# saurabh260918/Graph-Attention-Network-GATv2-

Hardware: AMD Instinct MI355X
Metric: edges/sec (fwd+bwd, 2-layer 8-head GATv2) (higher is better)
Workload: dtype f32; 1 GPU; products-shape synthetic power-law graph, 2450000 nodes / 61900000 edges / 100 feat / 47 classes, 2-layer GATv2 heads [8, 8] outdims [8, 8], fp32; launch=eager, parallelism=single GPU, generator=device (csrc/gat_synth.hip), bit-for-bit synth.py

## Files before the change

graph-attention-network-gatv2-_amd/csrc/gat_abi.hip:

```cpp
#include "gat_internal.h"

#include <algorithm>
#include <cmath>
#include <cstdlib>
#include <cstring>
#include <memory>
#include <mutex>

namespace gat {

static thread_local std::string g_err;
void set_error(const std::string& msg) { g_err = msg; }
int fail(int code, const std::string& msg) {
    g_err = msg;
    return code ? code : GAT_E_INVALID;
}
static std::mutex g_choice_mu;
static std::vector<std::pair<std::string, std::string>> g_choices;
const char* choice_env(const char* name) {
    const char* e = getenv(name);
    if (e) {
        std::lock_guard<std::mutex> lock(g_choice_mu);
        bool seen = false;
        for (auto& kv : g_choices) if (kv.first == name) { kv.second = e; seen = true; }
// ... 318 lines not shown
    if (c->drop_step) return 0;
    GAT_TRY(dalloc(c, &c->drop_step, 1));
    GAT_HIP(hipMemsetAsync(c->drop_step, 0, sizeof(uint64_t), c->stream));
    GAT_HIP(hipStreamSynchronize(c->stream));
    return 0;
}
static int32_t ldX_of(gat_ctx* c, int l) { return l == 0 ? c->ld0 : c->layers[l].F; }
static int upload_rows_padded(gat_ctx* c, float* dst, const float* src, int64_t n_rows, int32_t in_dim, hipMemcpyKind kind) {
    if (c->ld0 == in_dim) {
        GAT_HIP(hipMemcpyAsync(dst, src, (size_t)n_rows * in_dim * sizeof(float), kind, c->stream));
        return 0;
    }
    GAT_HIP(hipMemsetAsync(dst, 0, (size_t)n_rows * c->ld0 * sizeof(float), c->stream));
    GAT_HIP(hipMemcpy2DAsync(dst, (size_t)c->ld0 * sizeof(float), src, (size_t)in_dim * sizeof(float), (size_t)in_dim * sizeof(float), (size_t)n_rows, kind, c->stream));
    return 0;
}
static float* gPL_of(gat_ctx* c, int l) { return (c->ov_active && (l & 1)) ? c->gPL_alt : c->gPL; }
static float* gPR_of(gat_ctx* c, int l) { return (c->ov_active && (l & 1)) ? c->gPR_alt : c->gPR; }

static int ensure_drop_buffers(gat_ctx* c) {
    if (!c->buffers_ready || c->drop_pf <= 0.f) return 0;
    const int L = c->cfg.num_layers;
    if (c->xdrop.empty()) {
        c->xdrop.assign((size_t)L, nullptr);
        for (int l = 0; l < L; ++l) GAT_TRY(dalloc(c, &c->xdrop[(size_t)l], c->n_rows * (l == 0 ? c->ld0 : c->layers[l].F)));
    }
    if (c->Xtab && !c->xdrop_tab) GAT_TRY(dalloc(c, &c->xdrop_tab, c->n_table * c->ld0));
    return 0;
}
static int ensure_buffers(gat_ctx* c) {
    if (c->buffers_ready) return 0;
    if (!(c->have_graph && c->have_x && c->have_labels)) return 0;
    const int L = c->cfg.num_layers;
    const int64_t N = c->n_rows, E = c->n_edges, T = c->n_table;
    for (int l = 0; l < L; ++l) {
        Layer& y = c->layers[l];
        if (bf16(c) && !edge_fast_path(y.H, y.D, T))
            return fail(GAT_E_UNSUPPORTED, "bf16 storage needs every layer on the wave-per-row path (H*D in {8,16,32,64}, D a power of two)");
        if (!y.PL_bound) GAT_TRY(dmalloc(c, (void**)&y.PL, (size_t)(T * y.HD * st_bytes(c))));
        GAT_TRY(dalloc(c, &y.PR, N * y.HD));
        if (c->cfg.keep_taps || !edge_fast_path(y.H, y.D, c->n_table)) GAT_TRY(dalloc(c, &y.alpha, E * y.H));
        GAT_TRY(dalloc(c, &y.hpre, N * y.HD));
        GAT_TRY(dalloc(c, &y.hout, N * (l == L - 1 ? y.D : y.HD)));
        if (l < L - 1 || c->cfg.flat_lrelu_index) GAT_TRY(dalloc(c, &y.g, N * y.HD));
        GAT_TRY(dalloc(c, &y.mstat, N * y.H));
        GAT_TRY(dalloc(c, &y.zstat, N * y.H));
        if (c->cfg.keep_taps) {
            GAT_TRY(dalloc(c, &y.ge, E * y.H));
            GAT_TRY(dalloc(c, &y.score, E * y.H));
            GAT_TRY(dalloc(c, &y.galpha, E * y.H));
        }
    }
    if (!c->gPL_bound) GAT_TRY(dalloc(c, &c->gPL, T * c->HDmax));
    GAT_TRY(dalloc(c, &c->gPR, N * c->HDmax));
    if (!c->cfg.flat_lrelu_index) {
        const Layer& yl = c->layers[L - 1];
        const int w = edge_stash_words(yl.H, yl.D);
        c->gh_stride = (w > 0 && w <= 32 && yl.D <= 8 && !bf16(c) && !c->cfg.keep_taps) ? 16 : yl.D;
        GAT_TRY(dalloc(c, &c->gH, N * c->gh_stride));
    }
    GAT_TRY(dalloc(c, &c->items, std::max<int64_t>(c->work.n_items, 1)));
    GAT_TRY(dalloc(c, &c->slot_info, std::max<int32_t>(c->work.n_slots + c->work.n_split, 1)));
    GAT_TRY(dalloc(c, &c->part_acc, (int64_t)std::max<int32_t>(c->work.n_slots, 1) * c->HDmax));
    GAT_TRY(dalloc(c, &c->part_mz, (int64_t)std::max<int32_t>(c->work.n_slots, 1) * 2 * c->Hmax));
    if (c->work.n_items > 0)
        GAT_HIP(hipMemcpyAsync(c->items, c->work.items.data(), c->work.items.size() * sizeof(int32_t),
                               hipMemcpyHostToDevice, c->stream));
    if (c->work.n_slots > 0)
        GAT_HIP(hipMemcpyAsync(c->slot_info, c->work.slot_info.data(), c->work.slot_info.size() * sizeof(int32_t),
                               hipMemcpyHostToDevice, c->stream));
    GAT_HIP(hipStreamSynchronize(c->stream));
    int32_t msg_hd = 0, stash_words = 0;
    const char* no_stash = choice_env("GAT_BWD_STASH");
    for (int l = 0; l < L; ++l) {
        Layer& y = c->layers[l];
        if (!edge_fast_path(y.H, y.D, c->n_table)) continue;
        const int w = edge_stash_words(y.H, y.D);
        y.stash = w > 0 && !c->cfg.keep_taps && !(no_stash && no_stash[0] == '0') && !(bf16(c) && y.HD < 64);
        if (y.stash) stash_words = std::max(stash_words, w); else msg_hd = std::max(msg_hd, y.HD);
    }
    const char* force = choice_env("GAT_BWD_ATOMICS");
    if ((msg_hd > 0 || stash_words > 0) && E > 0 && !(force && force[0] == '1')) {
        float* m = nullptr;
        int32_t *src_ptr = nullptr, *cdst = nullptr, *csrc = nullptr;
        if (hipMalloc((void**)&m, std::max<size_t>((size_t)(E + kPullPad) * msg_hd * (size_t)st_bytes(c), (size_t)(E + kPullPad) * stash_words * sizeof(uint32_t))) == hipSuccess) {
            c->owned.push_back(m);
            if (msg_hd > 0) { c->msg = m; c->msg_hd = msg_hd; }
            if (stash_words > 0) {
                c->stash = reinterpret_cast<uint32_t*>(m); c->stash_words = stash_words;
                if (msg_hd == 0) { c->msg = m; c->msg_hd = 0; }
                GAT_TRY(dalloc(c, &c->gfull, N * c->HDmax));
                if (c->layers[L - 1].stash && c->gH != nullptr && c->gh_stride == 16) c->hbits = reinterpret_cast<uint8_t*>(c->gH) + 32;
                GAT_TRY(dalloc(c, &cdst, E + kPullPad));
                GAT_HIP(hipMemsetAsync(cdst + E, 0, (size_t)kPullPad * sizeof(int32_t), c->stream));
                GAT_HIP(hipMemsetAsync(reinterpret_cast<uint32_t*>(m) + (size_t)E * stash_words, 0, (size_t)kPullPad * stash_words * sizeof(uint32_t), c->stream));
            }
            GAT_TRY(dalloc(c, &c->csc_pos, E));
            GAT_TRY(dalloc(c, &src_ptr, T + 1));
            static const int run_env = [] { const char* e = choice_env("GAT_PULL_RUN"); return e ? atoi(e) : -1; }();
            const int32_t run = run_env >= 0 ? (run_env / 32) * 32 : 64;
            if (run > 0) GAT_TRY(dalloc(c, &csrc, E + kPullPad));
            GAT_TRY(build_csc(c->col_idx, E, T, c->csc_pos, src_ptr, csrc, c->stream));
            if (cdst) GAT_TRY(build_csc_dst(c->row_ptr, c->csc_pos, cdst, N, E, c->stream));
            SourceIndex& ix = c->src_index;
            ix.src_ptr = src_ptr; ix.cdst = cdst; ix.n_table = T; ix.n_slots = E; ix.slot_capacity = E + kPullPad;
            HeavyList hl;
            GAT_TRY(build_heavy_list(src_ptr, T, E, &hl, c->stream, run));
            auto upload = [&](auto** d, const std::vector<int32_t>& h, int per) -> int {
                GAT_TRY(dalloc(c, d, std::max<int64_t>((int64_t)(h.size() / per), 1)));
                if (!h.empty()) GAT_HIP(hipMemcpyAsync(*d, h.data(), h.size() * sizeof(int32_t), hipMemcpyHostToDevice, c->stream));
                return 0;
            };
            if (hl.run > 0 && csrc != nullptr) {
                ix.run = hl.run; ix.n_runs = hl.n_runs; ix.n_open = (int32_t)(hl.open.size() / 4); ix.n_empty = (int64_t)hl.empty.size();
                int4* d_open = nullptr; int32_t* d_empty = nullptr;
                GAT_TRY(upload(&d_open, hl.open, 4));
                GAT_TRY(upload(&d_empty, hl.empty, 1));
                GAT_TRY(dalloc(c, &ix.run_part, std::max<int64_t>(2 * ix.n_runs, 1) * c->HDmax));
                GAT_HIP(hipStreamSynchronize(c->stream));
                ix.open = d_open; ix.empty = d_empty; ix.csrc = csrc;
            }
            ix.n_chunks = (int32_t)(hl.chunks.size() / 4); ix.n_heavy = (int32_t)(hl.heavy.size() / 4);
            if (c->stash != nullptr && !hl.items.empty()) {
                int4* d_items = nullptr;
                GAT_TRY(upload(&d_items, hl.items, 4));
                GAT_HIP(hipStreamSynchronize(c->stream));
                ix.items = d_items; ix.n_items = (int64_t)(hl.items.size() / 4);
            }
            if (ix.n_heavy > 0) {
                int4* d_chunks = nullptr; int4* d_heavy = nullptr;
                GAT_TRY(upload(&d_chunks, hl.chunks, 4));
                GAT_TRY(upload(&d_heavy, hl.heavy, 4));
                GAT_TRY(dalloc(c, &ix.part, (int64_t)ix.n_chunks * c->HDmax));
                GAT_HIP(hipStreamSynchronize(c->stream));
                ix.chunks = d_chunks; ix.heavy = d_heavy;
            }
        } else {
            (void)hipGetLastError();
            for (int l = 0; l < L; ++l) c->layers[l].stash = false;
        }
    } else {
        for (int l = 0; l < L; ++l) c->layers[l].stash = false;
    }
    GAT_TRY(dalloc(c, &c->ga_partial, (int64_t)L * kGaPartialRows * c->HDmax));
    int64_t gw = 0;
    c->gw_off.assign((size_t)L, 0);
    for (int l = 0; l < L; ++l) { c->gw_off[(size_t)l] = gw; gw += grad_w_scratch_floats(N, c->layers[l].F, c->layers[l].HD); }
    gw = std::max<int64_t>(gw, 1);
    if (c->Xtab) gw = std::max(gw, grad_w_scratch_floats(T, c->layers[0].F, c->layers[0].HD));
    for (int l = 0; l < L; ++l) {
        const Layer& y = c->layers[l];
        if (l == 0 && c->Xtab) gw = std::max({gw, project_scratch_floats(T, y.F, y.HD, kPartLeft), project_scratch_floats(N, y.F, y.HD, kPartRight)});
        else gw = std::max(gw, project_scratch_floats(N, y.F, y.HD, kPartBoth));
    }
    GAT_TRY(dalloc(c, &c->gw_scratch, gw));
    c->gw_scratch_floats = gw;
    const int C = c->cfg.num_classes, DL = c->layers[L - 1].D;
    const int64_t NH = head_rows(c);
    GAT_TRY(dalloc(c, &c->hb_partial, (int64_t)head_bwd_blocks(NH, C, DL) * C * DL));
    GAT_TRY(dalloc(c, &c->loss_partial, head_blocks(NH)));
    GAT_TRY(dalloc(c, &c->correct_partial, head_blocks(NH)));
    GAT_TRY(dalloc(c, &c->loss_out, 1));
    GAT_TRY(dalloc(c, &c->correct_out, 1));
    GAT_TRY(dalloc(c, &c->y, NH * C));
    if (res_route(c)) {
        if (norm_on(c)) GAT_TRY(dalloc(c, &c->norm_partial, (int64_t)L * 2 * kResPartialRows * c->HDmax));
        GAT_TRY(dalloc(c, &c->resG, N * c->HDmax));
        GAT_TRY(dalloc(c, &c->res_agg, N * c->HDmax));
        GAT_TRY(dalloc(c, &c->res_partial, (int64_t)L * kResPartialRows * c->HDmax));
        if (c->group_cnt[GAT_PARAM_WRES]) {
            int64_t rg = 0;
            c->res_gw_off.assign((size_t)L, 0);
            for (int l = 0; l < L; ++l) {
                GAT_TRY(dalloc(c, &c->layers[l].R, N * c->layers[l].HD));
                c->res_gw_off[(size_t)l] = rg;
                rg += grad_w_scratch_floats(N, c->layers[l].F, c->layers[l].HD);
            }
            GAT_TRY(dalloc(c, &c->res_gw_scratch, std::max<int64_t>(rg, 1)));
        }
        GAT_TRY(ensure_drop_step(c));
    }
    if (edge_feat_on(c)) {
        const int64_t Ea = std::max<int64_t>(E, 1);
        int64_t wg = 0;
        c->we_gw_off.assign((size_t)L, 0);
        for (int l = 0; l < L; ++l) {
            GAT_TRY(dalloc(c, &c->layers[l].PE, Ea * c->layers[l].HD));
            c->we_gw_off[(size_t)l] = wg;
// ... 574 lines not shown
    }
    float* own_rows = reinterpret_cast<float*>(reinterpret_cast<char*>(y.PL) + c->table_row0 * y.HD * st_bytes(c));
    return launch_project(Xin_of(c, l), W_of(c, l), own_rows, y.PR, c->n_rows, y.F, y.HD, kPartBoth, bf16(c), c->gw_scratch, c->gw_scratch_floats, c->stream, ldX_of(c, l));
}

static EdgeFwdArgs plan_forward_edges(gat_ctx* c, int32_t l);
int gat_layer_forward_edges(gat_ctx* c, int32_t l) {
    GAT_TRY(check_layer(c, l));
    GAT_TRY(check_edge_features(c));
    const EdgeFwdArgs a = plan_forward_edges(c, l);
    EdgeFwdExtras x;
    x.drop = drop_args(c, l); x.res = c->layers[l].R; x.bias = b_of(c, l); x.ln = ln_args(c, l); x.pe = c->layers[l].PE;
    Scope t(c, GAT_K_EDGE_FWD);
    return launch_edge_forward(a, c->stream, &x);
}
static EdgeFwdArgs plan_forward_edges(gat_ctx* c, int32_t l) {
    Layer& y = c->layers[l];
    EdgeFwdArgs a{};
    a.row_ptr = c->row_ptr; a.col_idx = c->col_idx; a.PL = y.PL; a.PR = y.PR; a.a = a_of(c, l);
    a.alpha = y.alpha; a.score = y.score; a.hpre = y.hpre; a.hout = y.hout; a.mstat = y.mstat; a.zstat = y.zstat;
    a.n_rows = c->n_rows; a.n_table = c->n_table; a.bf16 = bf16(c); a.H = y.H; a.D = y.D; a.is_last = (l == c->cfg.num_layers - 1);
    a.slope = c->cfg.negative_slope;
    a.items = c->items; a.n_items = c->work.n_items; a.slot_info = c->slot_info; a.n_slots = c->work.n_slots; a.n_split = c->work.n_split;
    a.part_acc = c->part_acc; a.part_mz = c->part_mz;
    return a;
}

static int readout_pool(gat_ctx* c) {
    if (!readout_on(c)) return 0;
    const Layer& y = c->layers.back();
    ReadoutFwdArgs a{};
    a.x = y.hout; a.x_stride = y.D; a.graph_ptr = c->ro_graph_ptr;
    a.items = c->ro_items; a.n_items = c->ro_n_items; a.split = c->ro_split; a.n_split = c->ro_n_split;
    a.pooled = c->ro_P; a.argmax = c->ro_argmax; a.part = c->ro_part; a.part_arg = c->ro_part_arg;
    a.width = y.D; a.mode = c->readout_mode;
    Scope t(c, GAT_K_HEAD_FWD);
    return launch_readout_forward(a, c->stream);
}
static int readout_unpool(gat_ctx* c) {
    if (!readout_on(c)) return 0;
    ReadoutBwdArgs a{};
    a.gpooled = c->ro_gP; a.argmax = c->ro_argmax; a.graph_ptr = c->ro_graph_ptr; a.node_graph = c->ro_node_graph;
    a.gh = c->gH; a.gh_stride = c->gh_stride; a.n_rows = c->n_rows;
    a.width = c->layers.back().D; a.mode = c->readout_mode;
    Scope t(c, GAT_K_HEAD_BWD);
    return launch_readout_backward(a, c->stream);
}
static void head_args(gat_ctx* c, HeadArgs* f, HeadBwdArgs* b);
static LossHeadArgs loss_head_args(gat_ctx* c);
int gat_head_forward(gat_ctx* c, float* loss_sum, int32_t* n_correct) {
    GAT_TRY(check_layer(c, 0));
    HeadArgs a{}; HeadBwdArgs unused{};
    head_args(c, &a, &unused);
    GAT_TRY(readout_pool(c));
    {
        Scope t(c, GAT_K_HEAD_FWD);
        if (c->loss_mode != 0) GAT_TRY(launch_loss_head_forward(loss_head_args(c), c->stream));
        else GAT_TRY(launch_head_forward(a, c->stream));
    }
    c->y_valid = true;
    if (loss_sum || n_correct) {
        float hl = 0.f; int32_t hc = 0;
        GAT_HIP(hipMemcpyAsync(&hl, c->loss_out, sizeof(float), hipMemcpyDeviceToHost, c->stream));
        GAT_HIP(hipMemcpyAsync(&hc, c->correct_out, sizeof(int32_t), hipMemcpyDeviceToHost, c->stream));
        GAT_HIP(hipStreamSynchronize(c->stream));
        if (loss_sum) *loss_sum = hl;
        if (n_correct) *n_correct = hc;
    }
    return 0;
}

int gat_head_backward(gat_ctx* c) {
    GAT_TRY(check_layer(c, 0));
    HeadArgs unused{}; HeadBwdArgs a{};
    head_args(c, &unused, &a);
    {
        Scope t(c, GAT_K_HEAD_BWD);
        if (c->loss_mode != 0) GAT_TRY(launch_loss_head_grad(loss_head_args(c), false, c->stream));
        else GAT_TRY(launch_head_backward(a, c->stream));
    }
    return readout_unpool(c);
}

struct BwdPlan { EdgeBwdArgs a; bool store, stash, last_g; DropArgs drop; };
static int plan_backward_edges(gat_ctx* c, int32_t l, BwdPlan* P) {
    Layer& y = c->layers[l];
    const bool store = c->msg != nullptr && edge_fast_path(y.H, y.D, c->n_table);
    const bool stash = store && y.stash && c->stash != nullptr;
    EdgeBwdArgs a{};
    a.row_ptr = c->row_ptr; a.col_idx = c->col_idx; a.PL = y.PL; a.PR = y.PR; a.a = a_of(c, l);
    a.alpha = y.alpha; a.mstat = y.mstat; a.zstat = y.zstat;
    a.hpre = y.hpre; a.g = y.g; a.gPL = gPL_of(c, l); a.gPR = gPR_of(c, l); a.ge = y.ge; a.galpha = y.galpha;
    a.g_raw = l < c->cfg.num_layers - 1;
    a.gh = (l == c->cfg.num_layers - 1) ? c->gH : nullptr; a.gh_stride = c->gh_stride; a.hb_stride = 64;
    if (res_route(c)) {
        a.g = c->resG; a.g_raw = 0; a.gh = nullptr; a.hpre = c->res_agg;
    }
    a.pos = store ? c->csc_pos : nullptr; a.msg = store ? c->msg : nullptr;
    a.stash = stash ? c->stash : nullptr; a.gfull = stash ? c->gfull : nullptr; a.stash_spare = (uint32_t)c->n_edges;
    static const int pull_last = [] { const char* e = choice_env("GAT_PULL_LAST"); return e ? (e[0] == '0' ? 0 : 1) : -1; }();
    const bool runs_form = c->src_index.csrc != nullptr && short_lists_take_runs(c->n_edges, c->n_table);
    const bool big_rows = (int64_t)c->n_rows * y.H * y.D * 4 > ((int64_t)(runs_form ? 64 : 128) << 20);
    const bool last_g = stash && a.gh != nullptr && c->hbits != nullptr && !bf16(c) && !edge_feat_on(c) && (pull_last >= 0 ? pull_last == 1 : big_rows) &&
                        c->n_rows < ((int64_t)1 << 26);
    a.hbits = last_g ? c->hbits : nullptr;
    a.items = c->items; a.n_items = c->work.n_items; a.slot_info = c->slot_info; a.n_slots = c->work.n_slots; a.n_split = c->work.n_split;
    a.part_acc = c->part_acc;
    a.dbg = c->dbg;
    a.ga_partial = c->ga_partial + (int64_t)l * kGaPartialRows * c->HDmax; a.n_rows = c->n_rows; a.n_table = c->n_table; a.bf16 = bf16(c); a.H = y.H; a.D = y.D;
    a.slope = c->cfg.negative_slope;
    P->drop = drop_args(c, l);
    a.ga_blocks = edge_backward_blocks(a, &P->drop, y.PE != nullptr);
    P->a = a; P->store = store; P->stash = stash; P->last_g = last_g;
    return 0;
}
static int sum_backward_edges(gat_ctx* c, int32_t l, const BwdPlan& P) {
    Layer& y = c->layers[l];
    if (!P.stash && !P.store) return 0;
    Scope t(c, GAT_K_GPL_SUM);
    if (P.stash) {
        const PullArgs p{c->stash, c->gfull, bf16(c), P.last_g ? c->gH : nullptr, P.last_g ? c->hbits : nullptr, c->gh_stride, 64,
                         a_of(c, l), c->cfg.negative_slope, gPL_of(c, l), y.H, y.D};
        return launch_gpl_pull(c->src_index, p, c->stream);
    }
    return launch_gpl_sum(c->src_index, c->msg, bf16(c), gPL_of(c, l), y.HD, c->stream);
}
static int res_backward_layer(gat_ctx* c, int32_t l) {
    Layer& y = c->layers[l];
    const bool last = l == c->cfg.num_layers - 1;
    ResBwdArgs r{};
    r.hpre = y.hpre; r.g = y.g; r.gh = (last && c->gH != nullptr) ? c->gH : nullptr; r.res = y.R; r.bias = b_of(c, l);
    r.G = c->resG; r.agg = c->res_agg;
    r.partial = b_of(c, l) ? c->res_partial + (int64_t)l * kResPartialRows * c->HDmax : nullptr;
    r.n_rows = c->n_rows; r.H = y.H; r.D = y.D; r.gh_stride = c->gh_stride; r.g_raw = last ? 0 : 1;
    r.slope = c->cfg.negative_slope;
    Scope t(c, GAT_K_MISC);
    if (norm_layer(c, l)) {
        NormBwdArgs n{};
        n.gamma = lng_of(c, l); n.beta = lnb_of(c, l); n.eps = c->norm_eps;
        n.part_gamma = c->norm_partial + (int64_t)l * 2 * kResPartialRows * c->HDmax;
        n.part_beta = n.part_gamma + (int64_t)kResPartialRows * c->HDmax;
        r.blocks = norm_backward_blocks(c->n_rows, y.HD);
        n.r = r;
        GAT_TRY(launch_norm_backward(n, c->stream));
        GAT_TRY(launch_reduce_partials_add(n.part_gamma, r.blocks, y.HD, glng_of(c, l), c->stream));
        GAT_TRY(launch_reduce_partials_add(n.part_beta, r.blocks, y.HD, glnb_of(c, l), c->stream));
    } else {
        r.blocks = res_backward_blocks(c->n_rows, y.HD);
        GAT_TRY(launch_res_backward(r, c->stream));
    }
    if (r.partial != nullptr) return launch_reduce_partials_add(r.partial, r.blocks, y.HD, gb_of(c, l), c->stream);
    return 0;
}
int gat_layer_backward_edges(gat_ctx* c, int32_t l) {
    GAT_TRY(check_layer(c, l));
    GAT_TRY(check_edge_features(c));
    Layer& y = c->layers[l];
    BwdPlan P;
    GAT_TRY(plan_backward_edges(c, l, &P));
    if (res_route(c)) GAT_TRY(res_backward_layer(c, l));
    if (!P.store) {
        Scope t(c, GAT_K_MISC);
        GAT_HIP(hipMemsetAsync(gPL_of(c, l), 0, (size_t)c->n_table * y.HD * sizeof(float), c->stream));
    }
    {
        Scope t(c, GAT_K_EDGE_BWD);
        GAT_TRY(launch_edge_backward(P.a, c->stream, &P.drop, y.PE, y.PE != nullptr ? c->gPE : nullptr));
    }
    GAT_TRY(sum_backward_edges(c, l, P));
    Scope t(c, GAT_K_MISC);
    return launch_reduce_partials_add(P.a.ga_partial, P.a.ga_blocks, y.HD, ga_of(c, l), c->stream);
}

static int backward_grad_w(gat_ctx* c, int32_t l, hipStream_t st) {
    Layer& y = c->layers[l];
    const float* gPL_rows = gPL_of(c, l) + c->table_row0 * y.HD;
    Scope t(c, GAT_K_GRAD_W, st);
    if (y.R != nullptr)
        GAT_TRY(launch_grad_wres(c->resG, Xin_of(c, l), gWres_of(c, l), c->res_gw_scratch + c->res_gw_off[(size_t)l], c->n_rows, y.F, y.HD, st, ldX_of(c, l)));
    if (y.PE != nullptr)
        GAT_TRY(launch_grad_wres(c->gPE, c->EA, gWe_of(c, l), c->we_gw_scratch + c->we_gw_off[(size_t)l], c->n_edges, c->edge_dim, y.HD, st, c->ea_ld));
    if (l == 0 && c->Xtab) {
        GAT_TRY(launch_grad_w(gPL_of(c, l), nullptr, Xtab_of(c), gW_of(c, l), c->gw_scratch, c->n_table, y.F, y.HD, kPartLeft, st, c->ld0));
        return launch_grad_w(nullptr, gPR_of(c, l), Xin_of(c, 0), gW_of(c, l), c->gw_scratch, c->n_rows, y.F, y.HD, kPartRight, st, c->ld0);
    }
    return launch_grad_w(gPL_rows, gPR_of(c, l), Xin_of(c, l), gW_of(c, l), c->gw_scratch + c->gw_off[(size_t)l], c->n_rows, y.F, y.HD, kPartBoth, st, ldX_of(c, l));
}
static int backward_grad_x(gat_ctx* c, int32_t l) {
    if (l == 0) return 0;
    Layer& y = c->layers[l];
    const float* gPL_rows = gPL_of(c, l) + c->table_row0 * y.HD;
    Scope t(c, GAT_K_GRAD_X);
    GAT_TRY(launch_grad_x(gPL_rows, gPR_of(c, l), W_of(c, l), nullptr, c->layers[l - 1].g, c->n_rows, y.F, y.HD,
                          c->cfg.negative_slope, c->stream));
    if (y.R != nullptr) GAT_TRY(launch_grad_x_res(c->resG, Wres_of(c, l), c->layers[l - 1].g, c->n_rows, y.F, y.HD, c->stream));
    if (feat_drop_on(c)) return launch_feat_drop_bwd(c->layers[l - 1].g, c->n_rows, y.F, drop_args(c, l, kDropFeat), c->stream);
    return 0;
}
int gat_layer_backward_dense(gat_ctx* c, int32_t l) {
    GAT_TRY(check_layer(c, l));
    GAT_TRY(check_edge_features(c));
    GAT_TRY(backward_grad_w(c, l, c->stream));
    return backward_grad_x(c, l);
}

// ... 1164 lines not shown
```

graph-attention-network-gatv2-_amd/csrc/gat_csc.hip:

```cpp
#include "gat_internal.h"

#include <hipcub/hipcub.hpp>
#include <utility>

namespace gat {
namespace {

__global__ __launch_bounds__(256) void iota_kernel(int32_t* v, int64_t n) {
    const int64_t stride = (int64_t)gridDim.x * blockDim.x;
    for (int64_t i = (int64_t)blockIdx.x * blockDim.x + threadIdx.x; i < n; i += stride) v[i] = (int32_t)i;
}
__global__ __launch_bounds__(256) void invert_perm_kernel(const int32_t* __restrict__ perm, int32_t* __restrict__ pos,
                                                         int64_t n) {
    const int64_t stride = (int64_t)gridDim.x * blockDim.x;
    for (int64_t i = (int64_t)blockIdx.x * blockDim.x + threadIdx.x; i < n; i += stride) pos[perm[i]] = (int32_t)i;
}
__global__ __launch_bounds__(256) void segment_offsets_kernel(const int32_t* __restrict__ keys, int64_t n_keys,
                                                             int32_t* __restrict__ ptr, int64_t n_seg) {
    const int64_t stride = (int64_t)gridDim.x * blockDim.x;
    for (int64_t s = (int64_t)blockIdx.x * blockDim.x + threadIdx.x; s <= n_seg; s += stride) {
        int64_t lo = 0, hi = n_keys;
        while (lo < hi) {
            const int64_t mid = (lo + hi) >> 1;
            if ((int64_t)keys[mid] < s) lo = mid + 1; else hi = mid;
// ... 226 lines not shown
}

template <int HD>
__global__ __launch_bounds__(256) void gpl_sum_bf16_group_kernel(const int32_t* __restrict__ src_ptr,
                                                                 const float* __restrict__ msg, float* __restrict__ gPL,
                                                                 int64_t n_table, int32_t kHeavySlots) {
    constexpr int LPR = HD / 8, RPI = 64 / LPR, U = 4;
    const int lane = threadIdx.x & 63;
    const int wave = __builtin_amdgcn_readfirstlane(threadIdx.x >> 6);
    const int q = lane % LPR, r = lane / LPR;
    const int64_t s = ((int64_t)blockIdx.x * 4 + wave) * RPI + r;
    int b = 0, e = 0;
    if (s < n_table) { b = src_ptr[s]; e = src_ptr[s + 1]; }
    const bool heavy = (e - b) > kHeavySlots;
    const bool big = !heavy && (e - b) > kGroupMax;
    const uint4* m8 = reinterpret_cast<const uint4*>(msg);
    float acc[8];
#pragma unroll
    for (int k = 0; k < 8; ++k) acc[k] = 0.f;
    auto add = [&](float (&a8)[8], const uint4& v) {
        const uint32_t w[4] = {v.x, v.y, v.z, v.w};
#pragma unroll
        for (int k = 0; k < 4; ++k) {
            a8[2 * k] += __builtin_bit_cast(float, w[k] << 16);
            a8[2 * k + 1] += __builtin_bit_cast(float, w[k] & 0xFFFF0000u);
        }
    };
    if (!big && !heavy) {
        for (int i0 = b; i0 < e; i0 += U) {
            uint4 v[U];
#pragma unroll
            for (int u = 0; u < U; ++u)
                v[u] = (i0 + u < e) ? m8[(int64_t)(i0 + u) * LPR + q] : make_uint4(0u, 0u, 0u, 0u);
#pragma unroll
            for (int u = 0; u < U; ++u) add(acc, v[u]);
        }
    }
    uint64_t todo = __ballot(big && q == 0);
    while (todo) {
        const int g = (__ffsll((unsigned long long)todo) - 1) / LPR;
        todo &= todo - 1;
        const int bg = __shfl(b, g * LPR), eg = __shfl(e, g * LPR);
        float t[8];
#pragma unroll
        for (int k = 0; k < 8; ++k) t[k] = 0.f;
        for (int i0 = bg; i0 < eg; i0 += RPI * U) {
            uint4 v[U];
#pragma unroll
            for (int u = 0; u < U; ++u) {
                const int i = i0 + u * RPI + r;
                v[u] = (i < eg) ? m8[(int64_t)i * LPR + q] : make_uint4(0u, 0u, 0u, 0u);
            }
#pragma unroll
            for (int u = 0; u < U; ++u) add(t, v[u]);
        }
#pragma unroll
        for (int off = LPR; off < 64; off <<= 1)
#pragma unroll
            for (int k = 0; k < 8; ++k) t[k] += __shfl_xor(t[k], off);
        if (r == g) {
#pragma unroll
            for (int k = 0; k < 8; ++k) acc[k] = t[k];
        }
    }
    if (s < n_table && !heavy) {
        float4* out = reinterpret_cast<float4*>(gPL + s * HD + q * 8);
        out[0] = make_float4(acc[0], acc[1], acc[2], acc[3]);
        out[1] = make_float4(acc[4], acc[5], acc[6], acc[7]);
    }
}

template <int N> struct PullVec;
template <> struct PullVec<2> { typedef float T __attribute__((ext_vector_type(2))); };
template <> struct PullVec<4> { typedef float T __attribute__((ext_vector_type(4))); };

template <class T>
__device__ __forceinline__ void stream_store(T* p, const T& v) {
#ifdef GAT_NT_STORES
    __builtin_nontemporal_store(v, p);
#else
    *p = v;
#endif
}
template <int HD, int N, bool BF, int LASTD>
__device__ __forceinline__ typename PullVec<N>::T pull_range(const uint32_t* __restrict__ stash,
                                                             const int32_t* __restrict__ cdst,
                                                             const float* __restrict__ gfull, const uint8_t* __restrict__ hbits, int gh_stride, int hb_stride,
                                                             float slope, int b, int e, int lane,
                                                             typename PullVec<N>::T ac, typename PullVec<N>::T acs) {
    using V = typename PullVec<N>::T;
    constexpr int LPE = HD / N, G = 64 / LPE;
    constexpr int CH = 16, U = CH / G;
    static_assert(U >= 1, "lane layout");
    const int cp = lane % LPE, gidx = lane / LPE;
    V acc;
#pragma unroll
    for (int i = 0; i < N; ++i) acc[i] = 0.f;
    auto load_dst = [&](int i0) {
        const int j = i0 + (lane & (CH - 1));
        return cdst[j < e ? j : e - 1];
    };
    int dv = load_dst(b);
    for (int i0 = b; i0 < e; i0 += CH) {
        const int dn = (i0 + CH < e) ? load_dst(i0 + CH) : 0;
        uint32_t w[U];
        V g[U];
#pragma unroll
        for (int u = 0; u < U; ++u) {
            const int i = i0 + u * G + gidx;
            const int ic = i < e ? i : e - 1;
            w[u] = stash[(uint64_t)(uint32_t)ic * LPE + cp];
            const uint32_t drow = (uint32_t)__shfl(dv, u * G + gidx);
            if constexpr (LASTD > 0) {
                constexpr float inv_heads = 1.0f / (float)(HD / LASTD);
                const V gh4 = *reinterpret_cast<const V*>(gfull + (size_t)drow * gh_stride + (cp * N) % LASTD);
                const uint32_t nib = hbits[(size_t)drow * hb_stride + cp];
#pragma unroll
                for (int k = 0; k < N; ++k) g[u][k] = gh4[k] * ((nib >> k) & 1u ? 1.0f : slope) * inv_heads;
            } else if constexpr (BF) {
                const char* p = reinterpret_cast<const char*>(gfull) + drow * (uint32_t)(HD * 2) + (uint32_t)cp * (uint32_t)(N * 2);
                if constexpr (N == 2) {
                    const uint32_t w2 = *reinterpret_cast<const uint32_t*>(p);
                    g[u][0] = __builtin_bit_cast(float, w2 << 16); g[u][1] = __builtin_bit_cast(float, w2 & 0xFFFF0000u);
                } else {
                    const uint2 w2 = *reinterpret_cast<const uint2*>(p);
                    g[u][0] = __builtin_bit_cast(float, w2.x << 16); g[u][1] = __builtin_bit_cast(float, w2.x & 0xFFFF0000u);
                    g[u][2] = __builtin_bit_cast(float, w2.y << 16); g[u][3] = __builtin_bit_cast(float, w2.y & 0xFFFF0000u);
                }
            } else {
                const uint32_t off = drow * (uint32_t)(HD * 4) + (uint32_t)cp * (uint32_t)(N * 4);
#ifdef GAT_NT_GATHER
                g[u] = __builtin_nontemporal_load(reinterpret_cast<const V*>(reinterpret_cast<const char*>(gfull) + off));
#else
                g[u] = *reinterpret_cast<const V*>(reinterpret_cast<const char*>(gfull) + off);
#endif
            }
        }
#pragma unroll
        for (int u = 0; u < U; ++u) {
            const int i = i0 + u * G + gidx;
            const float val = __builtin_bit_cast(float, w[u] & ~((1u << N) - 1u));
            const float oth = __shfl_xor(val, 1);
            const float al = (cp & 1) ? oth : val, ge = (cp & 1) ? val : oth;
            V asel;
#pragma unroll
            for (int k = 0; k < N; ++k) asel[k] = (w[u] >> k) & 1u ? ac[k] : acs[k];
            const float keep = i < e ? 1.0f : 0.0f;
            acc += (g[u] * al + asel * ge) * keep;
        }
        dv = dn;
    }
#pragma unroll
    for (int off = LPE; off < 64; off <<= 1)
#pragma unroll
        for (int k = 0; k < N; ++k) acc[k] += __shfl_xor(acc[k], off);
    return acc;
}

template <int N> struct PullTabs { alignas(16) float m[2][1 << N][N]; };
template <int N>
__device__ __forceinline__ void pull_tabs_init(PullTabs<N>& T, float slope, float inv_heads) {
    for (int t = threadIdx.x; t < 2 * (1 << N) * N; t += blockDim.x) {
        const int tab = t / ((1 << N) * N), nib = (t / N) % (1 << N), k = t % N;
        const float v = (nib >> k) & 1 ? 1.0f : slope;
        T.m[tab][nib][k] = tab ? v * inv_heads : v;
    }
    __syncthreads();
}
template <int K>
__device__ __forceinline__ float select_bit(uint32_t bits, float a, float b) {
    uint32_t mask, sel;
    asm("v_bfe_i32 %0, %1, %2, 1" : "=v"(mask) : "v"(bits), "n"(K));
    asm("v_bfi_b32 %0, %1, %2, %3" : "=v"(sel) : "v"(mask), "v"(__builtin_bit_cast(uint32_t, a)), "v"(__builtin_bit_cast(uint32_t, b)));
    return __builtin_bit_cast(float, sel);
}
template <int N>
__device__ __forceinline__ typename PullVec<N>::T select_bits(uint32_t bits, typename PullVec<N>::T a, typename PullVec<N>::T b) {
    typename PullVec<N>::T r;
    r[0] = select_bit<0>(bits, a[0], b[0]);
    r[1] = select_bit<1>(bits, a[1], b[1]);
    if constexpr (N > 2) { r[2] = select_bit<2>(bits, a[2], b[2]); r[3] = select_bit<3>(bits, a[3], b[3]); }
    return r;
}
template <int HD, int N, int LASTD, bool TAB>
__device__ __forceinline__ typename PullVec<N>::T pull_range2(const PullTabs<N>& T, const uint32_t* __restrict__ stash,
                                                              const int32_t* __restrict__ cdst, const float* __restrict__ gfull,
                                                              const uint8_t* __restrict__ hbits, int b, int e, int lane,
                                                              typename PullVec<N>::T ac, float slope) {
    using V = typename PullVec<N>::T;
    [[maybe_unused]] const V acs = ac * slope;
    [[maybe_unused]] V mhi, mlo;
    if constexpr (LASTD > 0) {
#pragma unroll
        for (int k = 0; k < N; ++k) { mhi[k] = 1.0f / (float)(HD / LASTD); mlo[k] = slope * (1.0f / (float)(HD / LASTD)); }
    }
    constexpr int LPE = HD / N, G = 64 / LPE;
    constexpr int CH = 16, U = CH / G;
    constexpr uint32_t kMask = (1u << N) - 1u;
    static_assert(U >= 1, "lane layout");
    const int cp = lane % LPE, gidx = lane / LPE;
    V acc;
#pragma unroll
    for (int i = 0; i < N; ++i) acc[i] = 0.f;
    const char* sp = reinterpret_cast<const char*>(stash + (uint64_t)(uint32_t)b * LPE);
    const char* dp = reinterpret_cast<const char*>(cdst + b);
    const uint32_t doff = (uint32_t)(lane & (CH - 1)) * 4u;
    int dv = *reinterpret_cast<const int32_t*>(dp + doff);
    for (int rem = e - b; rem > 0; rem -= CH, sp += CH * LPE * 4, dp += CH * 4) {
        const int dn = *reinterpret_cast<const int32_t*>(dp + CH * 4 + doff);
        const int d0 = __builtin_amdgcn_readfirstlane(dv);
        uint32_t w[U];
        V g[U];
#pragma unroll
        for (int u = 0; u < U; ++u) {
            const bool valid = u * G + gidx < rem;
            const uint32_t ww = *reinterpret_cast<const uint32_t*>(sp + (uint32_t)((u * G + gidx) * LPE + cp) * 4u);
            int drow = __shfl(dv, u * G + gidx);
            drow = valid ? drow : d0;
            w[u] = valid ? ww : 0u;
            if constexpr (LASTD > 0) {
                const uint32_t ro = (uint32_t)drow << 6;
                const V gh4 = *reinterpret_cast<const V*>(reinterpret_cast<const char*>(gfull) + (ro + (uint32_t)((cp * N) % LASTD) * 4u));
                const uint32_t nib = *reinterpret_cast<const uint8_t*>(reinterpret_cast<const char*>(hbits) + (ro + (uint32_t)cp));
                if constexpr (TAB) g[u] = gh4 * *reinterpret_cast<const V*>(&T.m[1][nib & kMask][0]);
                else g[u] = gh4 * select_bits<N>(nib, mhi, mlo);
            } else {
                g[u] = *reinterpret_cast<const V*>(reinterpret_cast<const char*>(gfull) + ((uint32_t)drow * (uint32_t)(HD * 4) + (uint32_t)cp * (uint32_t)(N * 4)));
            }
        }
#pragma unroll
        for (int u = 0; u < U; ++u) {
            const float val = __builtin_bit_cast(float, w[u] & ~kMask);
            const float oth = __builtin_bit_cast(float, __builtin_amdgcn_update_dpp(0, __builtin_bit_cast(int, val), 0xB1, 0xF, 0xF, true));
            const float al = (cp & 1) ? oth : val, ge = (cp & 1) ? val : oth;
            acc += g[u] * al;
            if constexpr (TAB) acc += (ac * ge) * *reinterpret_cast<const V*>(&T.m[0][w[u] & kMask][0]);
            else acc += select_bits<N>(w[u], ac, acs) * ge;
        }
        dv = dn;
    }
#pragma unroll
    for (int off = LPE; off < 64; off <<= 1)
#pragma unroll
        for (int k = 0; k < N; ++k) acc[k] += __shfl_xor(acc[k], off);
    return acc;
}

template <int HD, int N, bool BF, int LASTD, int V2 = 0>
__global__ __launch_bounds__(256) void gpl_pull_kernel(const int32_t* __restrict__ src_ptr, const uint32_t* __restrict__ stash,
                                                       const int32_t* __restrict__ cdst, const float* __restrict__ gfull,
                                                       const uint8_t* __restrict__ hbits, int gh_stride, int hb_stride,
                                                       const float* __restrict__ a, float slope, float* __restrict__ gPL,
                                                       int64_t n_table, int32_t kHeavySlots) {
    using V = typename PullVec<N>::T;
    constexpr int LPE = HD / N;
    __shared__ PullTabs<N> tabs;
    if constexpr (V2 == 1) pull_tabs_init<N>(tabs, slope, LASTD > 0 ? 1.0f / (float)(HD / (LASTD > 0 ? LASTD : 1)) : 1.0f);
    const int lane = threadIdx.x & 63;
    const int wave = __builtin_amdgcn_readfirstlane(threadIdx.x >> 6);
    const int64_t s = (int64_t)blockIdx.x * (blockDim.x >> 6) + wave;
    if (s >= n_table) return;
    const int b = __builtin_amdgcn_readfirstlane(src_ptr[s]), e = __builtin_amdgcn_readfirstlane(src_ptr[s + 1]);
    if (e - b > kHeavySlots) return;
    const int cp = lane % LPE;
    V acc;
    if (b < e) {
        const V ac = *reinterpret_cast<const V*>(a + cp * N);
        if constexpr (V2 != 0) acc = pull_range2<HD, N, LASTD, V2 == 1>(tabs, stash, cdst, gfull, hbits, b, e, lane, ac, slope);
        else acc = pull_range<HD, N, BF, LASTD>(stash, cdst, gfull, hbits, gh_stride, hb_stride, slope, b, e, lane, ac, ac * slope);
    } else {
#pragma unroll
        for (int i = 0; i < N; ++i) acc[i] = 0.f;
    }
    if (lane < LPE) stream_store(reinterpret_cast<V*>(gPL + s * HD + cp * N), acc);
}

template <int HD, int N, bool BF, int LASTD, int V2 = 0>
__global__ __launch_bounds__(256) void gpl_pull_chunk_kernel(const int4* __restrict__ chunks, int32_t n_chunks,
                                                             const uint32_t* __restrict__ stash, const int32_t* __restrict__ cdst,
                                                             const float* __restrict__ gfull, const uint8_t* __restrict__ hbits,
                                                             int gh_stride, int hb_stride, const float* __restrict__ a,
                                                             float slope, float* __restrict__ part) {
    using V = typename PullVec<N>::T;
    constexpr int LPE = HD / N;
    __shared__ PullTabs<N> tabs;
    if constexpr (V2 == 1) pull_tabs_init<N>(tabs, slope, LASTD > 0 ? 1.0f / (float)(HD / (LASTD > 0 ? LASTD : 1)) : 1.0f);
    const int lane = threadIdx.x & 63;
    const int wave = __builtin_amdgcn_readfirstlane(threadIdx.x >> 6);
    const int k = blockIdx.x * 4 + wave;
    if (k >= n_chunks) return;
    const int4 ch = chunks[k];
    const int cp = lane % LPE;
    const V ac = *reinterpret_cast<const V*>(a + cp * N);
    V acc;
    if constexpr (V2 != 0) acc = pull_range2<HD, N, LASTD, V2 == 1>(tabs, stash, cdst, gfull, hbits, __builtin_amdgcn_readfirstlane(ch.x), __builtin_amdgcn_readfirstlane(ch.y), lane, ac, slope);
    else acc = pull_range<HD, N, BF, LASTD>(stash, cdst, gfull, hbits, gh_stride, hb_stride, slope, ch.x, ch.y, lane, ac, ac * slope);
    if (lane < LPE) *reinterpret_cast<V*>(part + (int64_t)ch.z * HD + cp * N) = acc;
}

template <int HD, int N, bool BF, int LASTD>
__global__ __launch_bounds__(256) void gpl_pull3_kernel(const int4* __restrict__ items, int64_t n_items,
                                                        const uint32_t* __restrict__ stash, const int32_t* __restrict__ cdst,
                                                        const float* __restrict__ gfull, const uint8_t* __restrict__ hbits,
                                                        int gh_stride, int hb_stride,
                                                        const float* __restrict__ a, float slope, float* __restrict__ gPL,
                                                        float* __restrict__ part) {
    using V = typename PullVec<N>::T;
    constexpr int LPE = HD / N, G = 64 / LPE, U = 4;
    static_assert(LPE >= U, "lane layout");
    const int lane = threadIdx.x & 63;
    const int wave = __builtin_amdgcn_readfirstlane(threadIdx.x >> 6);
    const int cp = lane % LPE, gidx = lane / LPE;
    const int64_t it = ((int64_t)blockIdx.x * (blockDim.x >> 6) + wave) * G + gidx;
    int src = -1, b = 0, e = 0, pslot = -1;
    if (it < n_items) { const int4 item = items[it]; src = item.x; b = item.y; e = item.z; pslot = item.w; }
    const V ac = *reinterpret_cast<const V*>(a + cp * N);
    const V acs = ac * slope;
    V acc;
#pragma unroll
    for (int i = 0; i < N; ++i) acc[i] = 0.f;
    int nst = (e - b + U - 1) / U;
#pragma unroll
    for (int off = LPE; off < 64; off <<= 1) { const int o = __shfl_xor(nst, off); nst = nst > o ? nst : o; }
    nst = __builtin_amdgcn_readfirstlane(nst);
    auto load_dst = [&](int st) {
        int j = b + st * U + (cp & (U - 1));
        j = j < e ? j : e - 1;
        return cdst[j > 0 ? j : 0];
    };
    int dv = load_dst(0);
    for (int st = 0; st < nst; ++st) {
        const int dn = load_dst(st + 1);
        uint32_t w[U];
        V g[U];
#pragma unroll
        for (int u = 0; u < U; ++u) {
            int j = b + st * U + u;
            j = j < e ? j : e - 1;
            j = j > 0 ? j : 0;
            w[u] = stash[(uint64_t)(uint32_t)j * LPE + cp];
            const uint32_t drow = (uint32_t)__shfl(dv, gidx * LPE + u);
            if constexpr (LASTD > 0) {
                constexpr float inv_heads = 1.0f / (float)(HD / LASTD);
                const V gh4 = *reinterpret_cast<const V*>(gfull + (size_t)drow * gh_stride + (cp * N) % LASTD);
                const uint32_t nib = hbits[(size_t)drow * hb_stride + cp];
#pragma unroll
                for (int k = 0; k < N; ++k) g[u][k] = gh4[k] * ((nib >> k) & 1u ? 1.0f : slope) * inv_heads;
            } else if constexpr (BF) {
                const char* p = reinterpret_cast<const char*>(gfull) + drow * (uint32_t)(HD * 2) + (uint32_t)cp * (uint32_t)(N * 2);
                if constexpr (N == 2) {
                    const uint32_t w2 = *reinterpret_cast<const uint32_t*>(p);
                    g[u][0] = __builtin_bit_cast(float, w2 << 16); g[u][1] = __builtin_bit_cast(float, w2 & 0xFFFF0000u);
                } else {
                    const uint2 w2 = *reinterpret_cast<const uint2*>(p);
                    g[u][0] = __builtin_bit_cast(float, w2.x << 16); g[u][1] = __builtin_bit_cast(float, w2.x & 0xFFFF0000u);
                    g[u][2] = __builtin_bit_cast(float, w2.y << 16); g[u][3] = __builtin_bit_cast(float, w2.y & 0xFFFF0000u);
                }
            } else {
                const uint32_t off = drow * (uint32_t)(HD * 4) + (uint32_t)cp * (uint32_t)(N * 4);
#ifdef GAT_NT_GATHER
                g[u] = __builtin_nontemporal_load(reinterpret_cast<const V*>(reinterpret_cast<const char*>(gfull) + off));
#else
                g[u] = *reinterpret_cast<const V*>(reinterpret_cast<const char*>(gfull) + off);
#endif
            }
        }
#pragma unroll
        for (int u = 0; u < U; ++u) {
            const float val = __builtin_bit_cast(float, w[u] & ~((1u << N) - 1u));
            const float oth = __shfl_xor(val, 1);
            const float al = (cp & 1) ? oth : val, ge = (cp & 1) ? val : oth;
            V asel;
#pragma unroll
            for (int k = 0; k < N; ++k) asel[k] = (w[u] >> k) & 1u ? ac[k] : acs[k];
            const float keep = (b + st * U + u < e) ? 1.0f : 0.0f;
            acc += (g[u] * al + asel * ge) * keep;
        }
        dv = dn;
    }
    if (src < 0) return;
    float* dst = pslot < 0 ? gPL + (int64_t)src * HD : part + (int64_t)pslot * HD;
// ... 154 lines not shown
        }
        return;
    }
    const int64_t wv = (int64_t)((int)blockIdx.x - rd.zero_blocks) * 4 + wave;
    const int64_t r = wv * G + gidx;
    const int64_t j0 = r * rd.run, left = rd.n_slots - j0;
    const int cnt = left <= 0 ? 0 : (left < rd.run ? (int)left : rd.run);
    const int nT = (__builtin_amdgcn_readfirstlane(cnt) + SS - 1) / SS;
    if (nT == 0) return;
    const int64_t jb = cnt > 0 ? j0 : 0;
    const int sb = (cnt > 0 && j0 > 0) ? rd.csrc[j0 - 1] : -1;
    const char* mp = reinterpret_cast<const char*>(msg) + ((uint64_t)jb * LPR + q) * 16u;
    int code[K], coden[K], dummy;
#pragma unroll
    for (int k = 0; k < K; ++k) runs_index(rd, nullptr, jb, r, cnt, sb, 0, k * LPR + q, dummy, code[k]);
    for (int T = 0; T < nT; ++T, mp += SS * LPR * 16) {
#pragma unroll
        for (int k = 0; k < K; ++k) coden[k] = 0;
        if (T + 1 < nT) {
#pragma unroll
            for (int k = 0; k < K; ++k) runs_index(rd, nullptr, jb, r, cnt, sb, 0, (T + 1) * SS + k * LPR + q, dummy, coden[k]);
        }
        if (T * SS < cnt) {
            const int rem = cnt - T * SS;
            static_for(std::make_integer_sequence<int, SS / U>{}, [&](auto bc) {
                constexpr int b = decltype(bc)::value;
                uint4 v[U];
                static_for(std::make_integer_sequence<int, U>{}, [&](auto uc) {
                    constexpr int u = decltype(uc)::value, slot = b * U + u;
                    const uint4 vv = *reinterpret_cast<const uint4*>(mp + slot * LPR * 16);
                    v[u] = slot < rem ? vv : make_uint4(0u, 0u, 0u, 0u);
                });
                static_for(std::make_integer_sequence<int, U>{}, [&](auto uc) {
                    constexpr int u = decltype(uc)::value, slot = b * U + u;
                    const uint32_t w[4] = {v[u].x, v[u].y, v[u].z, v[u].w};
                    if constexpr (BF) {
#pragma unroll
                        for (int k = 0; k < 4; ++k) {
                            acc[2 * k] += __builtin_bit_cast(float, w[k] << 16);
                            acc[2 * k + 1] += __builtin_bit_cast(float, w[k] & 0xFFFF0000u);
                        }
                    } else {
#pragma unroll
                        for (int k = 0; k < 4; ++k) acc[k] += __builtin_bit_cast(float, w[k]);
                    }
                    const int cw = group_bcast<slot % LPR, LPR>(code[slot / LPR], gidx);
                    if (cw < 0) {
                        const uint32_t row = (uint32_t)cw & 0x7fffffffu;
                        store_row(row >= (uint32_t)rd.n_table ? rd.part + (size_t)(row - (uint32_t)rd.n_table) * HD : gPL + (size_t)row * HD);
#pragma unroll
                        for (int i = 0; i < CPL; ++i) acc[i] = 0.f;
                    }
                });
            });
        }
#pragma unroll
        for (int k = 0; k < K; ++k) code[k] = coden[k];
    }
}

__global__ __launch_bounds__(256) void gpl_runs_fix_kernel(const int4* __restrict__ open, int32_t n_open, const float* __restrict__ part,
                                                           float* __restrict__ gPL, int32_t Q ) {
    const int64_t t = (int64_t)blockIdx.x * blockDim.x + threadIdx.x;
    const int64_t k = t / Q;
    const int q = (int)(t % Q);
    if (k >= n_open) return;
    const int4 o = open[k];
    const float4* p4 = reinterpret_cast<const float4*>(part);
    float4 acc = p4[(int64_t)(2 * o.y + 1) * Q + q];
    int r = o.y + 1;
    for (; r + 4 <= o.z; r += 4) {
        float4 v[4];
#pragma unroll
        for (int i = 0; i < 4; ++i) v[i] = p4[(int64_t)(2 * (r + i) + 1) * Q + q];
#pragma unroll
        for (int i = 0; i < 4; ++i) { acc.x += v[i].x; acc.y += v[i].y; acc.z += v[i].z; acc.w += v[i].w; }
    }
    for (; r < o.z; ++r) { const float4 v = p4[(int64_t)(2 * r + 1) * Q + q]; acc.x += v.x; acc.y += v.y; acc.z += v.z; acc.w += v.w; }
    { const float4 v = p4[(int64_t)(2 * o.z) * Q + q]; acc.x += v.x; acc.y += v.y; acc.z += v.z; acc.w += v.w; }
    reinterpret_cast<float4*>(gPL)[(int64_t)o.x * Q + q] = acc;
}

__global__ __launch_bounds__(256) void csc_dst_kernel(const int32_t* __restrict__ row_ptr, const int32_t* __restrict__ pos,
                                                     int32_t* __restrict__ cdst, int64_t n_rows, int64_t n_edges) {
    const int64_t stride = (int64_t)gridDim.x * blockDim.x;
    for (int64_t e = (int64_t)blockIdx.x * blockDim.x + threadIdx.x; e < n_edges; e += stride) {
        int64_t lo = 0, hi = n_rows;
        while (hi - lo > 1) {
            const int64_t mid = (lo + hi) >> 1;
            if ((int64_t)row_ptr[mid] <= e) lo = mid; else hi = mid;
        }
        cdst[pos[e]] = (int32_t)lo;
    }
}

}

int build_csc_dst(const int32_t* row_ptr, const int32_t* pos, int32_t* cdst, int64_t n_rows, int64_t n_edges, hipStream_t s) {
    if (n_edges <= 0) return 0;
    const int64_t blocks = std::min<int64_t>((n_edges + 255) / 256, 65536);
    hipLaunchKernelGGL(csc_dst_kernel, dim3((unsigned)blocks), dim3(256), 0, s, row_ptr, pos, cdst, n_rows, n_edges);
    GAT_HIP(hipGetLastError());
    return 0;
}

static int pull_runs_env() {
    static const int v = [] { const char* e = choice_env("GAT_PULL_RUNS"); return e ? (e[0] == '0' ? 0 : 1) : -1; }();
    return v;
}
static int pull_groups_env() {
    static const int v = [] { const char* e = choice_env("GAT_PULL_GROUPS"); return e ? (e[0] == '1' ? 1 : 0) : -1; }();
    return v;
}
static int pull_u_env() {
    static const int v = [] { const char* e = choice_env("GAT_PULL_U"); return e ? atoi(e) : 0; }();
    return v;
}
static int pull_v2_env() {
    static const int v = [] { const char* e = choice_env("GAT_PULL_V2"); return e ? atoi(e) : -1; }();
    return v;
}
static int gpl_waves_env() {
    static const int v = [] { const char* e = choice_env("GAT_GPL_WAVES"); const int w = e ? atoi(e) : 0; return (w == 1 || w == 2 || w == 4) ? w : 0; }();
    return v;
}
static int gpl_group_env() {
    static const int v = [] { const char* e = choice_env("GAT_GPL_GROUP"); return e ? (e[0] == '1' ? 1 : 0) : -1; }();
    return v;
}
static int gpl_bf16_group_env() {
    static const int v = [] { const char* e = choice_env("GAT_GPL_BF16_GROUP"); return e ? (e[0] == '0' ? 0 : 1) : -1; }();
    return v;
}

namespace {
struct GplPick {
    enum Form { kLists, kItems, kRuns };
    const void* fn = nullptr;
    Form form = kLists;
    const void* chunk_fn = nullptr;
    unsigned grid = 0, block = 256;
    RunsDev rd{};
};
#define GAT_K(...) ((const void*)(__VA_ARGS__))

static GplPick pick_runs(const SourceIndex& ix, const void* fn, int G) {
    GplPick p{fn, GplPick::kRuns};
    RunsDev& rd = p.rd;
    rd.csrc = ix.csrc; rd.empty = ix.empty; rd.part = ix.run_part; rd.n_empty = ix.n_empty; rd.n_slots = ix.n_slots; rd.n_table = ix.n_table;
    rd.run = ix.run; rd.zero_blocks = (int32_t)((ix.n_empty + 4 * G * 8 - 1) / (4 * G * 8));
    const int64_t waves = (ix.n_runs + G - 1) / G;
    p.grid = (unsigned)(rd.zero_blocks + (waves + 3) / 4);
    return p;
}

template <int HD, int N, bool BF, int LASTD>
GplPick pick_pull(const SourceIndex& ix, const PullArgs& A, bool padded) {
    constexpr int LPE = HD / N, G = 64 / LPE;
    const int wpb = gpl_waves_env() ? gpl_waves_env() : 1;
    const int runs_env = pull_runs_env(), groups_env = pull_groups_env();
    const bool records64 = LASTD == 0 || (A.gh_stride == 16 && A.hb_stride == 64);
    const bool runs_ok = padded && ix.csrc != nullptr && ix.run % LPE == 0 && records64;
    if (runs_ok && (runs_env >= 0 ? runs_env == 1 : (groups_env < 0 && short_lists_take_runs(ix.n_slots, ix.n_table)))) {
        constexpr int U = LPE % 8 == 0 ? 8 : 4;
        const int u_env = pull_u_env();
        if constexpr (LPE == 16 && !BF) {
            if (u_env == 4) return pick_runs(ix, GAT_K(gpl_pull_runs_kernel<HD, N, BF, LASTD, 4>), G);
            if (u_env == 16) return pick_runs(ix, GAT_K(gpl_pull_runs_kernel<HD, N, BF, LASTD, 16>), G);
        }
        return pick_runs(ix, GAT_K(gpl_pull_runs_kernel<HD, N, BF, LASTD, U>), G);
    }
    const bool groups = groups_env >= 0 ? groups_env == 1 : (ix.n_slots < 8 * ix.n_table && ix.n_items >= 32768);
    if (ix.items != nullptr && groups) {
        const int64_t quads = (ix.n_items + G - 1) / G;
        return {GAT_K(gpl_pull3_kernel<HD, N, BF, LASTD>), GplPick::kItems, nullptr, (unsigned)((quads + 3) / 4)};
    }
    const int v2_env = pull_v2_env();
    const int v2_want = v2_env >= 0 ? v2_env : (LASTD > 0 ? 2 : 0);
    const int v2 = (padded && !BF && records64) ? v2_want : 0;
    const unsigned grid = (unsigned)((ix.n_table + wpb - 1) / wpb), block = 64u * wpb;
    if constexpr (!BF) {
        if (v2 == 1) return {GAT_K(gpl_pull_kernel<HD, N, BF, LASTD, 1>), GplPick::kLists, GAT_K(gpl_pull_chunk_kernel<HD, N, BF, LASTD, 1>), grid, block};
        if (v2 == 2) return {GAT_K(gpl_pull_kernel<HD, N, BF, LASTD, 2>), GplPick::kLists, GAT_K(gpl_pull_chunk_kernel<HD, N, BF, LASTD, 2>), grid, block};
    }
    return {GAT_K(gpl_pull_kernel<HD, N, BF, LASTD, 0>), GplPick::kLists, GAT_K(gpl_pull_chunk_kernel<HD, N, BF, LASTD, 0>), grid, block};
}

template <int HD>
GplPick pick_sum(const SourceIndex& ix, bool bf) {
    const int runs_env = pull_runs_env();
    const bool group_env = gpl_group_env() >= 0 || gpl_bf16_group_env() >= 0;
    if (ix.csrc != nullptr && ix.run % 16 == 0 &&
        (runs_env >= 0 ? runs_env == 1 : (!group_env && !bf && short_lists_take_runs(ix.n_slots, ix.n_table))))
        return pick_runs(ix, bf ? GAT_K(gpl_sum_runs_kernel<HD, true>) : GAT_K(gpl_sum_runs_kernel<HD, false>), 64 / (HD / (bf ? 8 : 4)));
    const int wpb = gpl_waves_env() ? gpl_waves_env() : 4;
    const unsigned wgrid = (unsigned)((ix.n_table + wpb - 1) / wpb), wblock = 64u * wpb;
    const int rpi = 64 / (HD / (bf ? 8 : 4));
    const unsigned ggrid = (unsigned)((ix.n_table + 4 * rpi - 1) / (4 * rpi));
    if (bf) {
        const void* chunk = GAT_K(gpl_chunk_kernel<HD, true>);
        if (gpl_bf16_group_env() != 0) return {GAT_K(gpl_sum_bf16_group_kernel<HD>), GplPick::kLists, chunk, ggrid};
        return {GAT_K(gpl_sum_bf16_kernel<HD>), GplPick::kLists, chunk, wgrid, wblock};
    }
    const void* chunk = GAT_K(gpl_chunk_kernel<HD, false>);
    const int force = gpl_group_env();
    const bool group = force >= 0 ? force == 1 : ix.n_slots < 8 * ix.n_table;
    if (group) return {GAT_K(gpl_sum_group_kernel<HD>), GplPick::kLists, chunk, ggrid};
    return {GAT_K(gpl_sum_kernel<HD>), GplPick::kLists, chunk, wgrid, wblock};
}

}

static GplPick pick_pull_pass(const SourceIndex& ix, const PullArgs& A, bool last, bool padded) {
#define GAT_PULL_SHAPE(HD_, N_, D_)                                                                      \
    case HD_ * 1000 + D_:                                                                                \
        if (last) return pick_pull<HD_, N_, false, D_>(ix, A, padded);                                   \
        return A.g_bf16 ? pick_pull<HD_, N_, true, 0>(ix, A, padded) : pick_pull<HD_, N_, false, 0>(ix, A, padded);
    switch (A.H * A.D * 1000 + A.D) {
        GAT_PULL_SHAPE(64, 4, 8) GAT_PULL_SHAPE(32, 4, 8) GAT_PULL_SHAPE(64, 2, 4) GAT_PULL_SHAPE(32, 2, 4) GAT_PULL_SHAPE(16, 2, 4) GAT_PULL_SHAPE(8, 2, 4)
        default: return {};
    }
#undef GAT_PULL_SHAPE
}
static GplPick pick_sum_pass(const SourceIndex& ix, int32_t HD, bool bf) {
    switch (HD) {
        case 64: return pick_sum<64>(ix, bf);
        case 32: return pick_sum<32>(ix, bf);
        case 16: return pick_sum<16>(ix, bf);
        case 8: return pick_sum<8>(ix, bf);
        default: return {};
    }
}

static int run_pick(const SourceIndex& ix, const GplPick& p, void** args, void** chunk_args, float* gPL, int32_t HD, hipStream_t s) {
    const bool heavy = p.form != GplPick::kRuns && ix.n_heavy > 0;
    auto heavy_fix = [&] {
        const int64_t threads = (int64_t)ix.n_heavy * HD;
        hipLaunchKernelGGL(gpl_heavy_fix_kernel, dim3((unsigned)((threads + 255) / 256)), dim3(256), 0, s, ix.heavy, ix.n_heavy, ix.part, gPL, HD);
    };
    if (heavy && p.chunk_fn != nullptr) {
        GAT_HIP(hipLaunchKernel(p.chunk_fn, dim3((unsigned)((ix.n_chunks + 3) / 4)), dim3(256), chunk_args, 0, s));
        heavy_fix();
    }
    if (p.grid > 0) GAT_HIP(hipLaunchKernel(p.fn, dim3(p.grid), dim3(p.block), args, 0, s));
    if (heavy && p.chunk_fn == nullptr) heavy_fix();
    if (p.form == GplPick::kRuns && ix.n_open > 0) {
        const int64_t threads = (int64_t)ix.n_open * (HD / 4);
        hipLaunchKernelGGL(gpl_runs_fix_kernel, dim3((unsigned)((threads + 255) / 256)), dim3(256), 0, s, ix.open, ix.n_open, ix.run_part, gPL, HD / 4);
    }
    GAT_HIP(hipGetLastError());
    return 0;
}

int launch_gpl_pull(const SourceIndex& ix, const PullArgs& A, hipStream_t s) {
    if (ix.n_table <= 0) return 0;
    const bool padded = ix.slot_capacity >= ix.n_slots + kPullPad;
    const bool last = A.gh != nullptr && A.hbits != nullptr;
    GplPick p = pick_pull_pass(ix, A, last, padded);
    if (p.fn == nullptr) return fail(GAT_E_UNSUPPORTED, "gpl_pull: no stash path for this (H, D)");
    SourceIndex x = ix;
    PullArgs q = A;
    const float* g = last ? A.gh : A.gfull;
    int32_t hs = heavy_slots(ix.n_slots);
    void* lists[] = {&x.src_ptr, &q.stash, &x.cdst, &g, &q.hbits, &q.gh_stride, &q.hb_stride, &q.a, &q.slope, &q.gPL, &x.n_table, &hs};
    void* chunk[] = {&x.chunks, &x.n_chunks, &q.stash, &x.cdst, &g, &q.hbits, &q.gh_stride, &q.hb_stride, &q.a, &q.slope, &x.part};
    void* items[] = {&x.items, &x.n_items, &q.stash, &x.cdst, &g, &q.hbits, &q.gh_stride, &q.hb_stride, &q.a, &q.slope, &q.gPL, &x.part};
    void* runs[] = {&q.stash, &x.cdst, &g, &q.hbits, &q.a, &q.slope, &q.gPL, &p.rd};
    return run_pick(ix, p, p.form == GplPick::kRuns ? runs : p.form == GplPick::kItems ? items : lists, chunk, A.gPL, A.H * A.D, s);
}

int build_csc(const int32_t* col_idx, int64_t n_edges, int64_t n_table, int32_t* pos, int32_t* src_ptr,
              int32_t* csrc, hipStream_t s) {
    if (csrc) GAT_HIP(hipMemsetAsync(csrc + std::max<int64_t>(n_edges, 0), 0xFF, (size_t)kPullPad * sizeof(int32_t), s));
    if (n_edges <= 0) {
        GAT_HIP(hipMemsetAsync(src_ptr, 0, (size_t)(n_table + 1) * sizeof(int32_t), s));
        return 0;
    }
    int32_t *iota = nullptr, *keys_out = nullptr, *perm = nullptr;
    void* temp = nullptr;
    size_t temp_bytes = 0;
    int end_bit = 1;
    while (((int64_t)1 << end_bit) < n_table) ++end_bit;
    int rc = 0;
    auto cleanup = [&]() { (void)hipFree(iota); (void)hipFree(keys_out); (void)hipFree(perm); (void)hipFree(temp); };
#define CSC_HIP(x) do { hipError_t e__ = (x); if (e__ != hipSuccess) { cleanup(); return fail((int)e__, std::string(#x) + ": " + hipGetErrorString(e__)); } } while (0)
    CSC_HIP(hipMalloc((void**)&iota, n_edges * sizeof(int32_t)));
    CSC_HIP(hipMalloc((void**)&keys_out, n_edges * sizeof(int32_t)));
    CSC_HIP(hipMalloc((void**)&perm, n_edges * sizeof(int32_t)));
    int64_t blocks = std::min<int64_t>((n_edges + 255) / 256, 65536);
    hipLaunchKernelGGL(iota_kernel, dim3((unsigned)blocks), dim3(256), 0, s, iota, n_edges);
    CSC_HIP(hipcub::DeviceRadixSort::SortPairs(nullptr, temp_bytes, col_idx, keys_out, iota, perm, (int)n_edges, 0,
                                               end_bit, s));
    CSC_HIP(hipMalloc(&temp, temp_bytes));
    CSC_HIP(hipcub::DeviceRadixSort::SortPairs(temp, temp_bytes, col_idx, keys_out, iota, perm, (int)n_edges, 0,
                                               end_bit, s));
    hipLaunchKernelGGL(invert_perm_kernel, dim3((unsigned)blocks), dim3(256), 0, s, perm, pos, n_edges);
    if (csrc) CSC_HIP(hipMemcpyAsync(csrc, keys_out, (size_t)n_edges * sizeof(int32_t), hipMemcpyDeviceToDevice, s));
    const int64_t sblocks = std::min<int64_t>((n_table + 1 + 255) / 256, 65536);
    hipLaunchKernelGGL(segment_offsets_kernel, dim3((unsigned)sblocks), dim3(256), 0, s, keys_out, n_edges, src_ptr,
                       n_table);
    CSC_HIP(hipGetLastError());
    CSC_HIP(hipStreamSynchronize(s));
#undef CSC_HIP
    cleanup();
    return rc;
}

int build_heavy_list(const int32_t* d_src_ptr, int64_t n_table, int64_t n_edges, HeavyList* out, hipStream_t s, int32_t run) {
    out->chunks.clear(); out->heavy.clear();
    out->run = 0; out->n_runs = 0; out->open.clear(); out->empty.clear();
    if (n_table <= 0) return 0;
    std::vector<int32_t> ptr((size_t)n_table + 1);
    GAT_HIP(hipMemcpyAsync(ptr.data(), d_src_ptr, ptr.size() * sizeof(int32_t), hipMemcpyDeviceToHost, s));
    GAT_HIP(hipStreamSynchronize(s));
    if (run > 0 && n_table + 2 * ((n_edges + run - 1) / run) + 2 < 0x7fffffffLL) {
        out->run = run; out->n_runs = (n_edges + run - 1) / run;
        for (int64_t src = 0; src < n_table; ++src) {
            const int32_t b = ptr[(size_t)src], e = ptr[(size_t)src + 1];
            if (e == b) { out->empty.push_back((int32_t)src); continue; }
            const int32_t r0 = b / run, r1 = (e - 1) / run;
            if (r0 != r1) out->open.insert(out->open.end(), {(int32_t)src, r0, r1, 0});
        }
    }
    const int kHeavySlots = heavy_slots(n_edges);
    out->threshold = kHeavySlots;
    out->items.clear();
    for (int64_t src = 0; src < n_table; ++src) {
        const int32_t b = ptr[(size_t)src], e = ptr[(size_t)src + 1];
        if (e - b <= kHeavySlots) continue;
        const int32_t first = (int32_t)(out->chunks.size() / 4);
        int32_t n = 0;
        for (int32_t cb = b; cb < e; cb += kHeavySlots, ++n) {
            out->chunks.insert(out->chunks.end(), {cb, std::min(e, cb + kHeavySlots), first + n, 0});
            out->items.insert(out->items.end(), {(int32_t)src, cb, std::min(e, cb + kHeavySlots), first + n});
        }
        out->heavy.insert(out->heavy.end(), {(int32_t)src, first, n, 0});
    }
    {
        const int64_t win = 4096;
        std::vector<int64_t> cnt((size_t)kHeavySlots + 2);
        for (int64_t s0 = 0; s0 < n_table; s0 += win) {
            const int64_t s1 = std::min(n_table, s0 + win);
            std::fill(cnt.begin(), cnt.end(), 0);
            for (int64_t sr = s0; sr < s1; ++sr) { const int32_t d = ptr[(size_t)sr + 1] - ptr[(size_t)sr]; if (d <= kHeavySlots) ++cnt[(size_t)(kHeavySlots - d) + 1]; }
            for (size_t i = 1; i < cnt.size(); ++i) cnt[i] += cnt[i - 1];
            const size_t base = out->items.size();
            out->items.resize(base + 4 * (size_t)cnt.back());
            for (int64_t sr = s0; sr < s1; ++sr) {
// ... 24 lines not shown
```

graph-attention-network-gatv2-_amd/csrc/gat_edge_kernels.hip:

```cpp
#include "gat_internal.h"

#include <algorithm>
#include <map>
#include <mutex>
#include <utility>

namespace gat {
namespace {

constexpr float kLog2e = 1.4426950408889634f;
constexpr float kLn2 = 0.6931471805599453f;

__device__ __forceinline__ float lrelu(float v, float s) { return v > 0.f ? v : v * s; }
__device__ __forceinline__ float exp2_fast(float x) { return __builtin_amdgcn_exp2f(x); }
__device__ __forceinline__ float attn_keep(const DropArgs& d, uint32_t kd, int k, int h) {
    return drop_factor(d, drop_mix(drop_mix(kd, (uint32_t)k), (uint32_t)h));
}
__device__ __forceinline__ uint32_t edge_row_key(const DropArgs& d, int64_t row) { return drop_mix(drop_edge_key(d), drop_node(d, row)); }
struct RowKeys { uint32_t kd, ke; int rb; };
__device__ __forceinline__ void row_keys(const DropArgs& d, int64_t row, const int32_t* row_ptr, RowKeys& k) {
    k.kd = drop_mix(drop_key(d, kDropAttn), drop_node(d, row)); k.rb = row_ptr[row]; k.ke = edge_row_key(d, row);
}
__device__ __forceinline__ float pe_load(const float* __restrict__ pe, int j, int HD, int c) { return pe[(int64_t)j * HD + c]; }
template <bool EXT> struct FwdArgsOf { typedef EdgeFwdArgs T; };
// ... 458 lines not shown
        }
#pragma unroll
        for (int off = HD; off < 64; off <<= 1) gpr += __shfl_xor(gpr, off);
        if (gidx == 0) {
            if (slot < 0) A.gPR[row * HD + c] = gpr;
            else A.part_acc[(int64_t)slot * HD + c] = gpr;
        }
    }
#pragma unroll
    for (int off = HD; off < 64; off <<= 1) ga += __shfl_xor(ga, off);
    if (gidx == 0) red[wave][c] = ga;
    __syncthreads();
    if (threadIdx.x < HD)
        A.ga_partial[(int64_t)blockIdx.x * HD + threadIdx.x] =
            (red[0][threadIdx.x] + red[1][threadIdx.x]) + (red[2][threadIdx.x] + red[3][threadIdx.x]);
}

template <int N> struct VecOf;
template <> struct VecOf<2> { typedef float T __attribute__((ext_vector_type(2))); };
template <> struct VecOf<4> { typedef float T __attribute__((ext_vector_type(4))); };
template <int N> using vnf = typename VecOf<N>::T;

template <int N> __device__ __forceinline__ vnf<N> vzero() {
    vnf<N> r;
#pragma unroll
    for (int i = 0; i < N; ++i) r[i] = 0.f;
    return r;
}
template <int N> __device__ __forceinline__ float hsum(vnf<N> v) {
    if constexpr (N == 2) return v[0] + v[1];
    else return (v[0] + v[1]) + (v[2] + v[3]);
}
template <int N> __device__ __forceinline__ vnf<N> lrelu_n(vnf<N> s, float slope) {
    const vnf<N> t = s * slope;
    vnf<N> r;
#pragma unroll
    for (int i = 0; i < N; ++i) r[i] = fmaxf(s[i], t[i]);
    return r;
}
template <int N> __device__ __forceinline__ vnf<N> select_pos(vnf<N> s, vnf<N> a, vnf<N> b) {
    vnf<N> r;
#pragma unroll
    for (int i = 0; i < N; ++i) r[i] = s[i] > 0.f ? a[i] : b[i];
    return r;
}
template <int N> __device__ __forceinline__ vnf<N> shfl_xor_n(vnf<N> v, int off) {
    vnf<N> r;
#pragma unroll
    for (int i = 0; i < N; ++i) r[i] = __shfl_xor(v[i], off);
    return r;
}

template <int HD, int N, bool BF>
__device__ __forceinline__ vnf<N> gather_row_n(const float* __restrict__ table, int row, int cp) {
    if constexpr (BF) {
        const uint32_t off = (uint32_t)row * (uint32_t)(HD * 2) + (uint32_t)cp * (uint32_t)(N * 2);
        const char* p = reinterpret_cast<const char*>(table) + off;
        vnf<N> r;
        if constexpr (N == 2) {
            const uint32_t w = *reinterpret_cast<const uint32_t*>(p);
            r[0] = __builtin_bit_cast(float, w << 16); r[1] = __builtin_bit_cast(float, w & 0xFFFF0000u);
        } else {
            const uint2 w = *reinterpret_cast<const uint2*>(p);
            r[0] = __builtin_bit_cast(float, w.x << 16); r[1] = __builtin_bit_cast(float, w.x & 0xFFFF0000u);
            r[2] = __builtin_bit_cast(float, w.y << 16); r[3] = __builtin_bit_cast(float, w.y & 0xFFFF0000u);
        }
        return r;
    } else {
        const uint32_t off = (uint32_t)row * (uint32_t)(HD * 4) + (uint32_t)cp * (uint32_t)(N * 4);
#ifdef GAT_NT_GATHER
        return __builtin_nontemporal_load(reinterpret_cast<const vnf<N>*>(reinterpret_cast<const char*>(table) + off));
#else
        return *reinterpret_cast<const vnf<N>*>(reinterpret_cast<const char*>(table) + off);
#endif
    }
}
template <class T>
__device__ __forceinline__ void stream_store(T* p, const T& v) {
#ifdef GAT_NT_STORES
    __builtin_nontemporal_store(v, p);
#else
    *p = v;
#endif
}
template <int HD, int N, bool BF>
__device__ __forceinline__ void store_row_n(float* __restrict__ msg, int slot, int cp, vnf<N> v) {
    if constexpr (BF) {
        char* p = reinterpret_cast<char*>(msg) + (uint64_t)(uint32_t)slot * (HD * 2) + cp * (N * 2);
        const uint32_t w0 = (uint32_t)f32_to_bf16(v[0]) | ((uint32_t)f32_to_bf16(v[1]) << 16);
        if constexpr (N == 2) *reinterpret_cast<uint32_t*>(p) = w0;
        else *reinterpret_cast<uint2*>(p) = make_uint2(w0, (uint32_t)f32_to_bf16(v[2]) | ((uint32_t)f32_to_bf16(v[3]) << 16));
    } else {
        char* p = reinterpret_cast<char*>(msg) + (uint64_t)(uint32_t)slot * (HD * 4) + cp * (N * 4);
        *reinterpret_cast<vnf<N>*>(p) = v;
    }
}

template <int N>
__device__ __forceinline__ vnf<N> pe_load_n(const float* __restrict__ pe, int j, int HD, int c) {
    return *reinterpret_cast<const vnf<N>*>(pe + (int64_t)j * HD + c);
}
template <int N>
__device__ __forceinline__ void gpe_store_n(float* __restrict__ gpe, int j, int HD, int c, vnf<N> gs) {
    stream_store(reinterpret_cast<vnf<N>*>(gpe + (int64_t)j * HD + c), gs);
}

template <int N>
__device__ __forceinline__ vnf<N> res_term_n(const EdgeFwdExtras& X, int64_t row, int HD, int c) {
    vnf<N> r = vzero<N>();
    if (X.res != nullptr) r = *reinterpret_cast<const vnf<N>*>(X.res + row * HD + c);
    if (X.bias != nullptr) r += *reinterpret_cast<const vnf<N>*>(X.bias + c);
    return r;
}

template <int HD, int N>
__device__ __forceinline__ vnf<N> ln_row_n(vnf<N> u, const LnArgs& ln, int c) {
    constexpr int LPE = HD / N;
    const vnf<N> d = u - row_lanes_sum<LPE>(hsum<N>(u)) * (1.0f / (float)HD);
    const float rstd = 1.0f / sqrtf(row_lanes_sum<LPE>(hsum<N>(d * d)) * (1.0f / (float)HD) + ln.eps);
    vnf<N> v;
#pragma unroll
    for (int i = 0; i < N; ++i) v[i] = ln.gamma[c + i] * (d[i] * rstd) + ln.beta[c + i];
    return v;
}

template <int HD, int D, int N, int UU, bool BF, bool EXT = false, bool PE = false, class AT = EdgeFwdArgs>
__device__ __forceinline__ void fwd2_chunk(const AT& A, int e0, int e_end_v, int cp, int gidx, int srcv,
                                           vnf<N> pr, vnf<N> ac2, float& m, float& Z, vnf<N>& acc, uint32_t kd = 0, int rb = 0,
                                           uint32_t ke = 0, int64_t row = 0) {
    constexpr int LPE = HD / N, G = 64 / LPE, DL = D / N;
    vnf<N> v[UU];
    [[maybe_unused]] bool ek[UU];
    [[maybe_unused]] vnf<N> pev[UU];
#pragma unroll
    for (int u = 0; u < UU; ++u) {
        const int src = __shfl(srcv, u * G + gidx);
        v[u] = gather_row_n<HD, N, BF>(A.PL, src, cp);
        if constexpr (PE) { const int j = e0 + u * G + gidx; pev[u] = pe_load_n<N>(A.x.pe, j < e_end_v ? j : e_end_v - 1, HD, N * cp); }
        if constexpr (EXT) ek[u] = drop_edge_kept(A.x.drop, ke, e0 + u * G + gidx - rb, src, row);
    }
    float t[UU];
#pragma unroll
    for (int u = 0; u < UU; ++u) {
        vnf<N> s = v[u] + pr;
        if constexpr (PE) s += pev[u];
        t[u] = hsum<N>(ac2 * lrelu_n<N>(s, A.slope));
    }
    group_sum_n<DL, UU>(t);
    float cm = -INFINITY;
#pragma unroll
    for (int u = 0; u < UU; ++u) {
        const int j = e0 + u * G + gidx;
        bool in = j < e_end_v;
        if constexpr (EXT) in = in && ek[u];
        t[u] = in ? t[u] : -INFINITY;
        cm = fmaxf(cm, t[u]);
    }
    const float mn = fmaxf(m, cm);
    const float scale = exp2_fast(m - mn);
    Z *= scale;
    acc = acc * scale;
#pragma unroll
    for (int u = 0; u < UU; ++u) {
        const float p = exp2_fast(t[u] - mn);
        Z += p;
        if constexpr (EXT) acc += (p * attn_keep(A.x.drop, kd, e0 + u * G + gidx - rb, (N * cp) / D)) * v[u];
// ... 285 lines not shown
#pragma unroll
    for (int i = 0; i < N; ++i) { one[i] = 1.0f; slp[i] = A.slope; }

    for (int64_t it = (int64_t)blockIdx.x * 4 + wave; it < A.n_items; it += nwaves) {
        const int4 item = A.items[it];
        const int64_t row = item.x;
        const int b = item.y, e_end = item.z, slot = item.w;
        const int e_end_v = per_lane(e_end);
        const vnf<N> hp = *reinterpret_cast<const vnf<N>*>(A.hpre + row * HD + c);
        const vnf<N> dsel = select_pos<N>(hp, one, slp);
        vnf<N> g;
        if (A.gh != nullptr) g = *reinterpret_cast<const vnf<N>*>(A.gh + row * A.gh_stride + (c % D)) * dsel * (1.0f / (float)H);
        else {
            g = *reinterpret_cast<const vnf<N>*>(A.g + row * HD + c);
            if (A.g_raw) g = g * dsel;
        }
        const vnf<N> pr = *reinterpret_cast<const vnf<N>*>(A.PR + row * HD + c);
        const float dot = group_sum<DL>(hsum<N>(g * hp));
        const float m2 = A.mstat[row * H + c / D];
        const float inv = __builtin_amdgcn_rcpf(A.zstat[row * H + c / D] + 1e-8f);
        vnf<N> gpr = vzero<N>();
        if constexpr (STASH) {
            if (gidx == 0 && (slot < 0 || b == A.row_ptr[row])) {
                if (A.hbits != nullptr) {
                    uint32_t nib = 0;
#pragma unroll
                    for (int i = 0; i < N; ++i) nib |= (hp[i] > 0.f ? 1u : 0u) << i;
                    A.hbits[row * A.hb_stride + cp] = (uint8_t)nib;
                } else {
                    *reinterpret_cast<vnf<N>*>(A.gfull + row * HD + c) = g;
                }
            }
        }
        auto load_idx = [&](int e0, int& srcv, int& posv) {
            const int jl = e0 + (lane & (CH - 1));
            const int jlc = jl < e_end ? jl : e_end - 1;
            srcv = A.col_idx[jlc];
            posv = (DBG == 2) ? jlc : A.pos[jlc];
        };
        int srcv = 0, posv = 0;
        if (b < e_end) load_idx(b, srcv, posv);
        RowKeys k{};
        if constexpr (DROP) row_keys(A.drop, row, A.row_ptr, k);
        for (int e0 = b; e0 < e_end; e0 += CH) {
            int srcn = 0, posn = 0;
            if (e0 + CH < e_end) load_idx(e0 + CH, srcn, posn);
            if constexpr (U >= 2) {
                if (e_end - e0 <= CH / 2) bwd2_chunk<HD, D, N, U / 2, DBG, BF, STASH, DROP, PE>(A, e0, e_end, e_end_v, cp, gidx, srcv, posv, g, pr, dot, ac, acs, ac2, m2, inv, ga, gpr, k.kd, k.rb, k.ke, row);
                else bwd2_chunk<HD, D, N, U, DBG, BF, STASH, DROP, PE>(A, e0, e_end, e_end_v, cp, gidx, srcv, posv, g, pr, dot, ac, acs, ac2, m2, inv, ga, gpr, k.kd, k.rb, k.ke, row);
            } else {
                bwd2_chunk<HD, D, N, U, DBG, BF, STASH, DROP, PE>(A, e0, e_end, e_end_v, cp, gidx, srcv, posv, g, pr, dot, ac, acs, ac2, m2, inv, ga, gpr, k.kd, k.rb, k.ke, row);
            }
            srcv = srcn; posv = posn;
        }
#pragma unroll
        for (int off = LPE; off < 64; off <<= 1) gpr += shfl_xor_n<N>(gpr, off);
        if (gidx == 0) {
            float* dst = slot < 0 ? A.gPR + row * HD + c : A.part_acc + (int64_t)slot * HD + c;
            *reinterpret_cast<vnf<N>*>(dst) = gpr;
        }
    }
#pragma unroll
    for (int off = LPE; off < 64; off <<= 1) ga += shfl_xor_n<N>(ga, off);
    if (gidx == 0) {
#pragma unroll
        for (int i = 0; i < N; ++i) red[wave][c + i] = ga[i];
    }
    __syncthreads();
    if (threadIdx.x < HD)
        A.ga_partial[(int64_t)blockIdx.x * HD + threadIdx.x] =
            (red[0][threadIdx.x] + red[1][threadIdx.x]) + (red[2][threadIdx.x] + red[3][threadIdx.x]);
}

template <int HD, int D, int N, int DBG = 0, bool BF = false, bool STASH = false, bool DROP = false, bool PE = false>
__global__ __launch_bounds__(256) void edge_bwd2_kernel(BwdArgsT<DROP> A) {
    static_assert(DROP || !PE, "the edge term travels in the extended argument struct");
    edge_bwd2_body<HD, D, N, DBG, BF, STASH, DROP, PE>(A);
}
template <int HD, int D, int N, int DBG = 0>
__global__ __launch_bounds__(256) __attribute__((amdgpu_waves_per_eu(4, 8))) void edge_bwd2s_kernel(EdgeBwdArgs A) {
    edge_bwd2_body<HD, D, N, DBG, false, true>(A);
}

template <int HD, int D, int N, int DBG = 0, bool BF = false, bool MSG = false, bool DROP = false, bool PE = false>
__global__ __launch_bounds__(256) __attribute__((amdgpu_waves_per_eu(DROP ? 3 : 4, 8))) void edge_bwd3_kernel(BwdArgsT<DROP> A) {
    static_assert(DROP || !PE, "the edge term travels in the extended argument struct");
    constexpr int LPE = HD / N, G = 64 / LPE, DL = D / N, H = HD / D;
    constexpr int U = 4;
    static_assert((MSG || DL == 2) && LPE >= U, "records: two lanes per head (one carries alpha, the other ge)");
    __shared__ float red[4][HD];
    const int lane = threadIdx.x & 63;
    const int wave = __builtin_amdgcn_readfirstlane(threadIdx.x >> 6);
    const int cp = lane % LPE, gidx = lane / LPE;
    const int c = N * cp;
    const vnf<N> ac = *reinterpret_cast<const vnf<N>*>(A.a + c);
    const vnf<N> acs = ac * A.slope;
    const vnf<N> ac2 = ac * kLog2e;
    const int64_t nquads = (A.n_items + G - 1) / G;
    const int64_t nwaves = (int64_t)gridDim.x * 4;
    vnf<N> ga = vzero<N>();
    [[maybe_unused]] uint32_t k1 = 0;
    [[maybe_unused]] uint32_t k1e = 0;
    if constexpr (DROP) { k1 = drop_key(A.drop, kDropAttn); k1e = drop_edge_key(A.drop); }

    for (int64_t q = (int64_t)blockIdx.x * 4 + wave; q < nquads; q += nwaves) {
        const int64_t it = q * G + gidx;
        int row = -1, b = 0, e = 0, slot = -1;
        if (it < A.n_items) { const int4 item = A.items[it]; row = item.x; b = item.y; e = item.z; slot = item.w; }
        const int64_t rowc = row < 0 ? 0 : row;
        auto load_idx = [&](int st, int& srcv, int& posv) {
            int j = b + st * U + (cp & (U - 1));
            j = j < e ? j : e - 1;
            j = j > 0 ? j : 0;
            srcv = A.col_idx[j];
            posv = (DBG == 2) ? j : A.pos[j];
            if constexpr (DBG >= 15 && DBG <= 18) {
                constexpr uint32_t K = DBG == 15 ? 64u : DBG == 16 ? 512u : DBG == 17 ? 4096u : 32768u;
                const uint32_t per = A.stash_spare / K;
                posv = (int)(((uint32_t)posv % K) * per + (uint32_t)j / K);
            }
        };
        auto spread = [&](int st, int srcv, int posv, int (&src)[U], uint32_t (&sl)[U]) {
#pragma unroll
            for (int u = 0; u < U; ++u) {
                src[u] = __shfl(srcv, gidx * LPE + u);
                uint32_t p = (uint32_t)__shfl(posv, gidx * LPE + u);
                if constexpr (DBG == 10) p &= (1u << 20) - 1u;
                if constexpr (DBG == 11) p &= (1u << 18) - 1u;
                if constexpr (DBG == 12) p &= (1u << 16) - 1u;
                if constexpr (DBG == 13) p &= (1u << 14) - 1u;
                if constexpr (DBG == 14) p &= (1u << 24) - 1u;
                sl[u] = (b + st * U + u < e) ? p : A.stash_spare;
            }
        };
        int srcv, posv, srcn, posn;
        load_idx(0, srcv, posv);
        load_idx(1, srcn, posn);
        const vnf<N> hp = *reinterpret_cast<const vnf<N>*>(A.hpre + rowc * HD + c);
        vnf<N> dsel;
#pragma unroll
        for (int i = 0; i < N; ++i) dsel[i] = hp[i] > 0.f ? 1.0f : A.slope;
        vnf<N> g;
        if (A.gh != nullptr) g = *reinterpret_cast<const vnf<N>*>(A.gh + rowc * A.gh_stride + (c % D)) * dsel * (1.0f / (float)H);
        else {
            g = *reinterpret_cast<const vnf<N>*>(A.g + rowc * HD + c);
            if (A.g_raw) g = g * dsel;
        }
        const vnf<N> pr = *reinterpret_cast<const vnf<N>*>(A.PR + rowc * HD + c);
        const float dot = group_sum<DL>(hsum<N>(g * hp));
        const float m2 = A.mstat[rowc * H + c / D];
        const float inv = __builtin_amdgcn_rcpf(A.zstat[rowc * H + c / D] + 1e-8f);
        [[maybe_unused]] uint32_t kd = 0;
        [[maybe_unused]] int kb = 0;
        [[maybe_unused]] uint32_t ke = 0;
        if constexpr (DROP) { const uint32_t nd = drop_node(A.drop, rowc); kd = drop_mix(k1, nd); ke = drop_mix(k1e, nd); kb = b - A.row_ptr[rowc]; }
        if (!MSG && row >= 0 && (slot < 0 || b == A.row_ptr[rowc])) {
            if (A.hbits != nullptr) {
                uint32_t nib = 0;
#pragma unroll
                for (int i = 0; i < N; ++i) nib |= (hp[i] > 0.f ? 1u : 0u) << i;
                A.hbits[rowc * A.hb_stride + cp] = (uint8_t)nib;
            } else {
                if constexpr (BF) store_row_n<HD, N, BF>(A.gfull, (int)rowc, cp, g);
                else stream_store(reinterpret_cast<vnf<N>*>(A.gfull + rowc * HD + c), g);
            }
        }
        vnf<N> gpr = vzero<N>();
        const int nst = wave_max_over_groups<HD, N>((e - b + U - 1) / U);
        if constexpr (DBG == 9) {
            float dummy = 0.f;
            int j0 = b + (cp & (U - 1));
            j0 = j0 < e ? j0 : e - 1;
            int sv = A.col_idx[j0 > 0 ? j0 : 0];
            for (int st = 0; st < nst; ++st) {
                int jn = b + (st + 1) * U + (cp & (U - 1));
                jn = jn < e ? jn : e - 1;
                const int sn = A.col_idx[jn > 0 ? jn : 0];
#pragma unroll
                for (int u = 0; u < U; ++u) {
                    const vnf<N> vv = gather_row_n<HD, N, BF>(A.PL, __shfl(sv, gidx * LPE + u), cp);
                    dummy += hsum<N>(vv);
                }
                sv = sn;
            }
            if (dummy == 12345.6789f) gpr[0] += 1.0f;
        }
        int src[U];
        uint32_t sl[U], pend_s[U], pend_w[U];
        [[maybe_unused]] vnf<N> pend_m[U];
        spread(0, srcv, posv, src, sl);
#pragma unroll
        for (int u = 0; u < U; ++u) { pend_w[u] = 0u; pend_s[u] = A.stash_spare; if constexpr (MSG) pend_m[u] = vzero<N>(); }
        for (int st = 0; st < nst; ++st) {
            vnf<N> v[U];
#pragma unroll
            for (int u = 0; u < U; ++u) v[u] = gather_row_n<HD, N, BF>(A.PL, src[u], cp);
            [[maybe_unused]] vnf<N> pev[U];
            if constexpr (PE) {
#pragma unroll
                for (int u = 0; u < U; ++u) {
                    int j = b + st * U + u;
                    j = j < e ? j : e - 1;
                    pev[u] = pe_load_n<N>(A.pe, j > 0 ? j : 0, HD, c);
                }
            }
            [[maybe_unused]] bool ek[U];
            if constexpr (DROP) {
#pragma unroll
                for (int u = 0; u < U; ++u) ek[u] = drop_edge_kept(A.drop, ke, kb + st * U + u, src[u], rowc);
            }
            if constexpr (MSG) {
                if constexpr (DBG != 1) {
#pragma unroll
                    for (int u = 0; u < U; ++u) store_row_n<HD, N, BF>(A.msg, (int)pend_s[u], cp, pend_m[u]);
                }
            } else if constexpr (DBG == 3) {
                const int j0 = b + (st > 0 ? st - 1 : 0) * U;
                uint4 w4 = make_uint4(pend_w[0], pend_w[1], pend_w[2], pend_w[3]);
                *reinterpret_cast<uint4*>(A.stash + (uint64_t)(uint32_t)(j0 < e ? j0 : 0) * LPE + cp * 4) = w4;
            } else if constexpr (DBG != 1) {
#pragma unroll
                for (int u = 0; u < U; ++u) stream_store(&A.stash[(uint64_t)pend_s[u] * LPE + cp], pend_w[u]);
            }
#pragma unroll
            for (int u = 0; u < U; ++u) pend_s[u] = sl[u];
            spread(st + 1, srcn, posn, src, sl);
            load_idx(st + 2, srcn, posn);
            float al[U], ga_[U];
#pragma unroll
            for (int u = 0; u < U; ++u) {
                vnf<N> s = v[u] + pr;
                if constexpr (PE) s += pev[u];
                al[u] = hsum<N>(ac2 * lrelu_n<N>(s, A.slope));
            }
            group_sum_n<DL, U>(al);
#pragma unroll
            for (int u = 0; u < U; ++u) {
                al[u] = exp2_fast(al[u] - m2) * inv;
                ga_[u] = hsum<N>(g * v[u]);
            }
            group_sum_n<DL, U>(ga_);
            [[maybe_unused]] bool kp[U];
            if constexpr (DROP) {
#pragma unroll
                for (int u = 0; u < U; ++u) {
                    kp[u] = ek[u] && (drop_mix(drop_mix(kd, (uint32_t)(kb + st * U + u)), (uint32_t)(c / D)) >> 8) >= A.drop.T;
                    ga_[u] = kp[u] ? ga_[u] * A.drop.scale : 0.f;
                }
            }
#pragma unroll
            for (int u = 0; u < U; ++u) {
                bool valid = b + st * U + u < e;
                if constexpr (DROP) valid = valid && ek[u];
                const float ge = valid ? al[u] * (ga_[u] - dot) : 0.f;
                vnf<N> s = v[u] + pr;
                if constexpr (PE) s += pev[u];
                const vnf<N> gs = ge * select_pos<N>(s, ac, acs);
                ga += ge * lrelu_n<N>(s, A.slope);
                gpr += gs;
                if constexpr (PE) { if (b + st * U + u < e) gpe_store_n<N>(A.gpe, b + st * U + u, HD, c, gs); }
                if constexpr (DROP) al[u] = kp[u] ? al[u] * A.drop.scale : 0.f;
                if constexpr (MSG) {
                    pend_m[u] = g * al[u] + gs;
                } else {
                    uint32_t bits = 0;
#pragma unroll
                    for (int i = 0; i < N; ++i) bits |= (s[i] > 0.f ? 1u : 0u) << i;
                    const uint32_t w = __builtin_bit_cast(uint32_t, (cp & 1) ? ge : al[u]);
                    pend_w[u] = ((w + (1u << (N - 1))) & ~((1u << N) - 1u)) | bits;
                }
            }
        }
        if constexpr (MSG) {
            if constexpr (DBG != 1) {
#pragma unroll
                for (int u = 0; u < U; ++u) store_row_n<HD, N, BF>(A.msg, (int)pend_s[u], cp, pend_m[u]);
            }
        } else if constexpr (DBG != 1 && DBG != 3) {
#pragma unroll
            for (int u = 0; u < U; ++u) stream_store(&A.stash[(uint64_t)pend_s[u] * LPE + cp], pend_w[u]);
        }
        if (row >= 0) {
            float* dst = slot < 0 ? A.gPR + rowc * HD + c : A.part_acc + (int64_t)slot * HD + c;
            stream_store(reinterpret_cast<vnf<N>*>(dst), gpr);
        }
    }
#pragma unroll
    for (int off = LPE; off < 64; off <<= 1) ga += shfl_xor_n<N>(ga, off);
    if (gidx == 0) {
#pragma unroll
        for (int i = 0; i < N; ++i) red[wave][c + i] = ga[i];
    }
    __syncthreads();
    if (threadIdx.x < HD)
        A.ga_partial[(int64_t)blockIdx.x * HD + threadIdx.x] =
            (red[0][threadIdx.x] + red[1][threadIdx.x]) + (red[2][threadIdx.x] + red[3][threadIdx.x]);
}

template <int HD, int D, int N>
__global__ __launch_bounds__(256) __attribute__((amdgpu_waves_per_eu(4, 8))) void edge_last_fused_kernel(EdgeLastArgs A) {
    constexpr int LPE = HD / N, G = 64 / LPE, DL = D / N, H = HD / D;
    constexpr int U = 4, JC = 4;
    static_assert(LPE == 16 && DL == 2 && D == 8 && N == 4, "16 lanes per row, two lanes per head, D = 8");
    __shared__ float red[4][HD];
    __shared__ float s_wo[64 * D];
    const EdgeFwdArgs& F = A.f;
    const EdgeBwdArgs& B = A.b;
    const int C = A.C;
    for (int i = threadIdx.x; i < C * D; i += blockDim.x) s_wo[i] = A.Wo[i];
    __syncthreads();
    const int lane = threadIdx.x & 63;
    const int wave = __builtin_amdgcn_readfirstlane(threadIdx.x >> 6);
    const int cp = lane % LPE, gidx = lane / LPE;
    const int c = N * cp;
    const vnf<N> ac = *reinterpret_cast<const vnf<N>*>(F.a + c);
    const vnf<N> acs = ac * F.slope;
    const vnf<N> ac2 = ac * kLog2e;
    const int64_t nquads = (F.n_items + G - 1) / G;
    const int64_t nwaves = (int64_t)gridDim.x * 4;
    vnf<N> ga = vzero<N>();

    for (int64_t q = (int64_t)blockIdx.x * 4 + wave; q < nquads; q += nwaves) {
        const int64_t it = q * G + gidx;
        int row = -1, b = 0, e = 0;
        if (it < F.n_items) { const int4 item = F.items[it]; row = item.x; b = item.y; e = item.z; }
        const int64_t rowc = row < 0 ? 0 : row;
        const int nst = wave_max_over_groups<HD, N>((e - b + U - 1) / U);
        const vnf<N> pr = *reinterpret_cast<const vnf<N>*>(F.PR + rowc * HD + c);
        float m = -1e9f * kLog2e, Z = 0.f;
        vnf<N> acc = vzero<N>();
        {
            auto load_src = [&](int st) {
                int j = b + st * U + (cp & (U - 1));
                j = j < e ? j : e - 1;
                return F.col_idx[j > 0 ? j : 0];
            };
            int srcv = load_src(0);
            for (int st = 0; st < nst; ++st) {
                const int srcn = load_src(st + 1);
                vnf<N> v[U];
#pragma unroll
                for (int u = 0; u < U; ++u) v[u] = gather_row_n<HD, N, false>(F.PL, __shfl(srcv, gidx * LPE + u), cp);
                float t[U];
#pragma unroll
                for (int u = 0; u < U; ++u) t[u] = hsum<N>(ac2 * lrelu_n<N>(v[u] + pr, F.slope));
                group_sum_n<DL, U>(t);
                float cm = -INFINITY;
#pragma unroll
                for (int u = 0; u < U; ++u) {
                    t[u] = (b + st * U + u < e) ? t[u] : -INFINITY;
                    cm = fmaxf(cm, t[u]);
                }
                const float mn = fmaxf(m, cm);
                const float scale = exp2_fast(m - mn);
                Z *= scale;
                acc = acc * scale;
#pragma unroll
                for (int u = 0; u < U; ++u) {
                    const float p = exp2_fast(t[u] - mn);
                    Z += p;
// ... 502 lines not shown
        return A.g_raw ? gv * (A.hpre[i] > 0.f ? 1.0f : slope) : gv;
    };
    const uint32_t k1 = dr.on ? drop_key(dr, kDropAttn) : 0u;
    const uint32_t k1e = dr.on ? drop_edge_key(dr) : 0u;
    for (int64_t row = blockIdx.x; row < A.n_rows; row += gridDim.x) {
        const int b = A.row_ptr[row], e_end = A.row_ptr[row + 1];
        const uint32_t kd = dr.on ? drop_mix(k1, drop_node(dr, row)) : 0u;
        const uint32_t ke = dr.on ? drop_mix(k1e, drop_node(dr, row)) : 0u;
        for (int h = lane; h < H; h += 64) {
            float t = 0.f;
            for (int k = 0; k < D; ++k) t += gval(row * HD + h * D + k) * A.hpre[row * HD + h * D + k];
            s_dot[h] = t;
        }
        for (int ch = lane; ch < HD; ch += 64) s_gpr[ch] = 0.f;
        __syncthreads();
        for (int e = b; e < e_end; ++e) {
            const int64_t sid = A.col_idx[e];
            if (dr.on && !drop_edge_kept(dr, ke, e - b, (int)sid, row)) {
                for (int h = lane; h < H; h += 64) {
                    if (A.ge != nullptr) A.ge[(int64_t)e * H + h] = 0.f;
                    if (A.galpha != nullptr) A.galpha[(int64_t)e * H + h] = 0.f;
                }
                if constexpr (PE) { for (int ch = lane; ch < HD; ch += 64) gpe[(int64_t)e * HD + ch] = 0.f; }
                continue;
            }
            for (int h = lane; h < H; h += 64) {
                float t = 0.f;
                for (int k = 0; k < D; ++k) t += gval(row * HD + h * D + k) * A.PL[sid * HD + h * D + k];
                const float al = A.alpha[(int64_t)e * H + h];
                const float kf = dr.on ? attn_keep(dr, kd, e - b, h) : 1.0f;
                t *= kf;
                const float ge = al * (t - s_dot[h]);
                s_ge[h] = ge;
                s_al[h] = al * kf;
                if (A.ge != nullptr) A.ge[(int64_t)e * H + h] = ge;
                if (A.galpha != nullptr) A.galpha[(int64_t)e * H + h] = t;
            }
            __syncthreads();
            for (int ch = lane; ch < HD; ch += 64) {
                const float v = A.PL[sid * HD + ch];
                float s = v + A.PR[row * HD + ch];
                if constexpr (PE) s += pe[(int64_t)e * HD + ch];
                const bool pos = s > 0.f;
                const float ge = s_ge[ch / D];
                const float gs = ge * A.a[ch] * (pos ? 1.0f : slope);
                s_ga[ch] += ge * (pos ? s : s * slope);
                s_gpr[ch] += gs;
                if constexpr (PE) gpe[(int64_t)e * HD + ch] = gs;
                unsafeAtomicAdd(A.gPL + sid * HD + ch, gval(row * HD + ch) * s_al[ch / D] + gs);
            }
            __syncthreads();
        }
        for (int ch = lane; ch < HD; ch += 64) A.gPR[row * HD + ch] = s_gpr[ch];
        __syncthreads();
    }
    for (int ch = lane; ch < HD; ch += 64) A.ga_partial[(int64_t)blockIdx.x * HD + ch] = s_ga[ch];
}
__global__ __launch_bounds__(64) void edge_bwd_generic(EdgeBwdArgs A, DropArgs dr) { edge_bwd_generic_body<false>(A, dr, nullptr, nullptr); }
__global__ __launch_bounds__(64) void edge_bwd_generic_pe(EdgeBwdArgs A, DropArgs dr, const float* pe, float* gpe) {
    edge_bwd_generic_body<true>(A, dr, pe, gpe);
}

__global__ __launch_bounds__(256) void transpose_kernel(const float* __restrict__ src,
                                                        float* __restrict__ dst, int64_t A_, int64_t B_) {
    const int64_t stride = (int64_t)gridDim.x * blockDim.x;
    const int64_t total = A_ * B_;
    for (int64_t i = (int64_t)blockIdx.x * blockDim.x + threadIdx.x; i < total; i += stride) {
        const int64_t a = i / B_, b = i % B_;
        dst[b * A_ + a] = src[i];
    }
}

#define GAT_EDGE_SHAPES(X, ...)                                                                                          \
    X(64, 8, __VA_ARGS__) X(64, 4, __VA_ARGS__) X(64, 16, __VA_ARGS__) X(64, 32, __VA_ARGS__) X(64, 64, __VA_ARGS__)    \
    X(32, 8, __VA_ARGS__) X(32, 4, __VA_ARGS__) X(32, 16, __VA_ARGS__) X(32, 32, __VA_ARGS__)                           \
    X(16, 4, __VA_ARGS__) X(16, 8, __VA_ARGS__) X(16, 16, __VA_ARGS__) X(8, 4, __VA_ARGS__) X(8, 8, __VA_ARGS__)
#define GAT_SHAPE_ENTRY(hd, d, ...) {hd, d},
constexpr struct { int HD, D; } kEdgeShapes[] = {GAT_EDGE_SHAPES(GAT_SHAPE_ENTRY)};
static_assert(sizeof(kEdgeShapes) / sizeof(kEdgeShapes[0]) == 14, "the wave-per-row kernels cover 14 shapes");
static bool edge_shape_listed(int HD, int D) {
    for (const auto& sh : kEdgeShapes) if (sh.HD == HD && sh.D == D) return true;
    return false;
}
constexpr int stash_n(int HD, int D) { return (D == 8 && HD >= 32) ? 4 : (D == 4 ? 2 : 0); }
template <int HD, int D> constexpr int stash_n() { return stash_n(HD, D); }

static bool row_groups() {
    static const bool v = [] { const char* e = choice_env("GAT_ROWGROUP"); return !(e && e[0] == '0'); }();
    return v;
}
static bool packed_layout() {
    static const bool v = [] { const char* e = choice_env("GAT_PACKED"); return !(e && e[0] == '0'); }();
    return v;
}
static int lane_channels() {
    static const int v = [] { const char* e = choice_env("GAT_CPL"); return (e && e[0] == '2') ? 2 : 4; }();
    return v;
}
static int fwd_waves() {
    static const int v = [] { const char* e = choice_env("GAT_FWD_WAVES"); const int w = e ? atoi(e) : 1; return (w == 1 || w == 2 || w == 4) ? w : 1; }();
    return v;
}
static bool group_msg() {
    static const bool v = [] { const char* e = choice_env("GAT_GROUP_MSG"); return !(e && e[0] == '0'); }();
    return v;
}

struct EdgePick {
    const void* fn = nullptr;
    unsigned block = 256;
    int per_block = 4;
    const void* fix = nullptr;
    int grid_div = 1;
};
#define GAT_K(...) ((const void*)(__VA_ARGS__))

template <int HD, int D, bool BF>
EdgePick pick_fwd(const EdgeFwdArgs& a, bool ext, bool res, bool pe) {
    static_assert(D % 2 == 0, "every fast-path shape has an even D");
    constexpr int N3 = stash_n<HD, D>(), N2 = (HD >= 32 && D % 4 == 0) ? 4 : 2;
    constexpr int G3 = N3 != 0 ? 64 / (HD / (N3 != 0 ? N3 : 1)) : 1;
    if (a.alpha != nullptr) {
        const void* fix = res ? GAT_K(edge_fwd_fix_kernel<HD, D, true, true>) : GAT_K(edge_fwd_fix_kernel<HD, D, true>);
        if (pe) return {GAT_K(edge_fwd_kernel<HD, D, true, BF, true, true>), 256, 4, fix};
        return {ext ? GAT_K(edge_fwd_kernel<HD, D, true, BF, true>) : GAT_K(edge_fwd_kernel<HD, D, true, BF>), 256, 4, fix};
    }
    const void* fix = res ? GAT_K(edge_fwd_fix_kernel<HD, D, false, true>) : GAT_K(edge_fwd_fix_kernel<HD, D, false>);
    if (pe) {
        if constexpr (N3 != 0) return {GAT_K(edge_fwd3_kernel<HD, D, N3, BF, true, true>), 64, G3, fix};
        else return {GAT_K(edge_fwd2_kernel<HD, D, N2, BF, true, true>), 64, 1, fix};
    }
    if (ext) {
        if constexpr (N3 != 0) return {GAT_K(edge_fwd3_kernel<HD, D, N3, BF, true>), 64, G3, fix};
        else return {GAT_K(edge_fwd2_kernel<HD, D, N2, BF, true>), 64, 1, fix};
    }
    if (!packed_layout()) return {GAT_K(edge_fwd_kernel<HD, D, false, BF>), 256, 4, fix};
    const int wpb = fwd_waves();
    if constexpr (N3 != 0) {
        if (row_groups()) return {GAT_K(edge_fwd3_kernel<HD, D, N3, BF>), 64u * wpb, G3 * wpb, fix};
    }
    if constexpr (N2 == 4) {
        if (lane_channels() == 4) return {GAT_K(edge_fwd2_kernel<HD, D, 4, BF>), 64u * wpb, wpb, fix};
    }
    return {GAT_K(edge_fwd2_kernel<HD, D, 2, BF>), 64u * wpb, wpb, fix};
}

#ifdef GAT_EXPERIMENTS
template <int... DBG>
const void* bwd3_dbg(int dbg) {
    const void* fn = nullptr;
    ((dbg == DBG ? (void)(fn = GAT_K(edge_bwd3_kernel<64, 8, 4, DBG>)) : (void)0), ...);
    return fn;
}
#endif

template <int HD, int D, bool BF>
EdgePick pick_bwd(const EdgeBwdArgs& a, bool drop, int dbg, bool pe) {
    constexpr int N3 = stash_n<HD, D>(), N2 = (HD >= 32 && D % 4 == 0) ? 4 : 2;
    const bool store = a.pos != nullptr && a.msg != nullptr, taps = a.ge != nullptr, stash = a.stash != nullptr && !taps;
    if (drop) {
        if (!store) return {};
        if (pe) {
            if (taps) return {GAT_K(edge_bwd_kernel<HD, D, true, true, 0, BF, true, true>)};
            if constexpr (N3 != 0) return {stash ? GAT_K(edge_bwd3_kernel<HD, D, N3, 0, BF, false, true, true>) : GAT_K(edge_bwd3_kernel<HD, D, N3, 0, BF, true, true, true>)};
            else return {GAT_K(edge_bwd2_kernel<HD, D, N2, 0, BF, false, true, true>)};
        }
        if (taps) return {GAT_K(edge_bwd_kernel<HD, D, true, true, 0, BF, true>)};
        if constexpr (N3 != 0) return {stash ? GAT_K(edge_bwd3_kernel<HD, D, N3, 0, BF, false, true>) : GAT_K(edge_bwd3_kernel<HD, D, N3, 0, BF, true, true>)};
        else return {GAT_K(edge_bwd2_kernel<HD, D, N2, 0, BF, false, true>)};
    }
    const bool msg_rows = store && !taps && packed_layout();
#ifdef GAT_EXPERIMENTS
    if constexpr (HD == 64 && D == 8) {
        if (store && !taps && !stash) {
            if (dbg == 1) return {GAT_K(edge_bwd_kernel<HD, D, true, false, 1>)};
            if (dbg == 2) return {GAT_K(edge_bwd_kernel<HD, D, true, false, 2>)};
        }
        if (stash && !BF && row_groups()) {
            if (const void* fn = bwd3_dbg<1, 2, 3, 9, 10, 11, 12, 13, 14, 15, 16, 17, 18>(dbg)) return {fn};
            if (dbg == 4) return {GAT_K(edge_bwd4_kernel<7, 4>), 512, 4, nullptr, 2};
            if (dbg == 5) return {GAT_K(edge_bwd4_kernel<3, 4>)};
            if (dbg == 6) return {GAT_K(edge_bwd4_kernel<3, 4, 1>)};
            if (dbg == 7) return {GAT_K(edge_bwd4_kernel<3, 4, 2>)};
            if (dbg == 8) return {GAT_K(edge_bwd4_kernel<3, 4, 3>)};
        } else if (stash && !BF) {
            if (dbg == 1) return {GAT_K(edge_bwd2s_kernel<64, 8, 4, 1>)};
            if (dbg == 2) return {GAT_K(edge_bwd2s_kernel<64, 8, 4, 2>)};
        }
    }
#endif
    if constexpr (N3 != 0) {
        if (stash) return {(BF || row_groups()) ? GAT_K(edge_bwd3_kernel<HD, D, N3, 0, BF>) : GAT_K(edge_bwd2s_kernel<HD, D, N3>)};
        if (msg_rows && row_groups() && group_msg()) {
#ifdef GAT_EXPERIMENTS
            if constexpr (HD == 32 && D == 8 && BF) {
                if (dbg == 1) return {GAT_K(edge_bwd3_kernel<HD, D, N3, 1, true, true>)};
            }
#endif
            return {GAT_K(edge_bwd3_kernel<HD, D, N3, 0, BF, true>)};
        }
    }
    if (msg_rows) {
        if constexpr (N2 == 4) {
            if (lane_channels() == 4) return {GAT_K(edge_bwd2_kernel<HD, D, 4, 0, BF>)};
        }
        return {GAT_K(edge_bwd2_kernel<HD, D, 2, 0, BF>)};
    }
    return {store ? (taps ? GAT_K(edge_bwd_kernel<HD, D, true, true, 0, BF>) : GAT_K(edge_bwd_kernel<HD, D, true, false, 0, BF>))
                  : (taps ? GAT_K(edge_bwd_kernel<HD, D, false, true, 0, BF>) : GAT_K(edge_bwd_kernel<HD, D, false, false, 0, BF>))};
}

#define GAT_SHAPE_CASE(hd, d, FN, BF, ...) case hd * 1000 + d: return (BF) ? FN<hd, d, true>(__VA_ARGS__) : FN<hd, d, false>(__VA_ARGS__);
#define GAT_DISPATCH_HD_D(HD, D, FN, BF, ...) \
    switch ((HD) * 1000 + (D)) { GAT_EDGE_SHAPES(GAT_SHAPE_CASE, FN, BF, __VA_ARGS__) default: break; }
static EdgePick pick_forward(const EdgeFwdArgs& a, bool ext, bool res, bool pe) {
    GAT_DISPATCH_HD_D(a.H * a.D, a.D, pick_fwd, a.bf16 != 0, a, ext, res, pe)
    return {};
}
static EdgePick pick_backward(const EdgeBwdArgs& a, bool drop, int dbg, bool pe = false) {
    GAT_DISPATCH_HD_D(a.H * a.D, a.D, pick_bwd, a.bf16 != 0, a, drop, dbg, pe)
    return {};
}

static int resident_blocks(const void* fn, unsigned block) {
    static std::mutex mu;
    static std::map<std::pair<const void*, unsigned>, int> cache;
    std::lock_guard<std::mutex> lock(mu);
    const auto key = std::make_pair(fn, block);
    auto it = cache.find(key);
    if (it != cache.end()) return it->second;
    int per_cu = 0, dev = 0, cus = 256;
    if (hipOccupancyMaxActiveBlocksPerMultiprocessor(&per_cu, fn, (int)block, 0) != hipSuccess || per_cu < 1) per_cu = 4;
    if (per_cu > 8) per_cu = 8;
    (void)hipGetDevice(&dev);
    (void)hipDeviceGetAttribute(&cus, hipDeviceAttributeMultiprocessorCount, dev);
    (void)hipGetLastError();
    return cache[key] = per_cu * (cus > 0 ? cus : 256);
}

static int launch_fwd_fix(const EdgePick& p, EdgeFwdExtArgs& a, hipStream_t s) {
    if (a.n_slots <= 0) return 0;
    const int64_t n = a.alpha != nullptr ? a.n_slots : a.n_split;
    void* args[] = {&a};
    GAT_HIP(hipLaunchKernel(p.fix, dim3((unsigned)((n + 3) / 4)), dim3(256), args, 0, s));
    return 0;
}
static int launch_bwd_fix(const EdgeBwdArgs& a, hipStream_t s) {
    if (a.n_slots <= 0) return 0;
    const int HD = a.H * a.D;
    const int64_t threads = (int64_t)a.n_split * HD;
    hipLaunchKernelGGL(edge_bwd_fix_kernel, dim3((unsigned)((threads + 255) / 256)), dim3(256), 0, s,
                       a.slot_info, a.n_slots, a.n_split, a.part_acc, a.gPR, HD);
    GAT_HIP(hipGetLastError());
    return 0;
}

constexpr int kGenericBlocks = 4096;

}

bool edge_fast_path(int32_t H, int32_t D, int64_t n_table) {
    return n_table * H * D * (int64_t)sizeof(float) < ((int64_t)1 << 32) && edge_shape_listed(H * D, D);
}
int edge_stash_words(int32_t H, int32_t D) {
    const int n = edge_shape_listed(H * D, D) ? stash_n(H * D, D) : 0;
    return n ? H * D / n : 0;
}

int launch_edge_forward(const EdgeFwdArgs& a, hipStream_t s, const EdgeFwdExtras* extras) {
    if (a.n_rows <= 0) return 0;
    EdgeFwdExtArgs ax;
    static_cast<EdgeFwdArgs&>(ax) = a;
    if (extras != nullptr) ax.x = *extras;
    EdgeFwdExtras& x = ax.x;
    if (x.ln.gamma == nullptr) x.ln = LnArgs{};
    else if (x.ln.beta == nullptr) return fail(GAT_E_INVALID, "edge_forward: layer normalisation without beta");
    const bool with_res = x.res != nullptr || x.bias != nullptr || x.ln.gamma != nullptr;
    if (!x.drop.on) { x.drop.T = 0; x.drop.Te = 0; x.drop.scale = 1.f; x.drop.eflags = 0; }
    if (edge_fast_path(a.H, a.D, a.n_table)) {
        if (a.items == nullptr) return fail(GAT_E_INVALID, "edge_forward: work-item list missing");
        if (a.mstat == nullptr || a.zstat == nullptr) return fail(GAT_E_INVALID, "edge_forward: stats buffers missing");
        const bool ext = with_res || x.drop.on != 0 || x.pe != nullptr;
        if (ext && x.drop.step == nullptr) return fail(GAT_E_INVALID, "edge_forward: extras without DropArgs::step (the extended kernels read the device counter)");
        const EdgePick p = pick_forward(a, ext, with_res, x.pe != nullptr);
        void* args[] = {&ax};
        GAT_HIP(hipLaunchKernel(p.fn, dim3((unsigned)((a.n_items + p.per_block - 1) / p.per_block)), dim3(p.block), args, 0, s));
        return launch_fwd_fix(p, ax, s);
    }
    const int HD = a.H * a.D;
    const int64_t blocks = a.n_rows < kGenericBlocks * 8 ? a.n_rows : kGenericBlocks * 8;
    void* args[] = {&ax, &x};
    GAT_HIP(hipLaunchKernel(x.pe != nullptr ? GAT_K(edge_fwd_generic_pe) : with_res ? GAT_K(edge_fwd_generic_res) : GAT_K(edge_fwd_generic), dim3((unsigned)blocks), dim3(64), args,
                            (size_t)HD * sizeof(float), s));
    return 0;
}

int edge_backward_blocks(const EdgeBwdArgs& a, const DropArgs* drop, bool pe) {
    if (!edge_fast_path(a.H, a.D, a.n_table))
        return (int)std::min<int64_t>(std::max<int64_t>(a.n_rows, 1), kGaPartialRows);
    const bool on = (drop != nullptr && drop->on != 0) || pe;
    EdgePick p = pick_backward(a, on, 0, pe);
    if (p.fn == nullptr) p = pick_backward(a, false, 0);
    int64_t cap = resident_blocks(p.fn, p.block);
#ifdef GAT_EXPERIMENTS
    cap /= pick_backward(a, on, a.dbg).grid_div;
#endif
    return (int)std::min({std::max<int64_t>((a.n_items + 3) / 4, 1), cap, (int64_t)kGaPartialRows});
}

int launch_edge_backward(const EdgeBwdArgs& a, hipStream_t s, const DropArgs* drop, const float* pe, float* gpe) {
    if (a.ga_blocks < 1) return fail(GAT_E_INVALID, "edge_backward: ga_blocks must come from edge_backward_blocks()");
    DropArgs dr = drop != nullptr ? *drop : DropArgs{};
    const bool with_pe = pe != nullptr;
    if (with_pe != (gpe != nullptr)) return fail(GAT_E_INVALID, "edge_backward: the edge term needs both PE and gPE");
    if (with_pe && !dr.on) { dr.T = 0; dr.Te = 0; dr.scale = 1.f; dr.eflags = 0; }
    const bool ext = dr.on != 0 || with_pe;
    if (edge_fast_path(a.H, a.D, a.n_table)) {
        if (a.items == nullptr) return fail(GAT_E_INVALID, "edge_backward: work-item list missing");
        if (a.stash != nullptr && a.ge == nullptr && (a.gfull == nullptr || a.pos == nullptr))
            return fail(GAT_E_INVALID, "edge_backward: stash path needs gfull and pos");
        if (ext && dr.step == nullptr) return fail(GAT_E_INVALID, "edge_backward: the extended kernels read the device counter (DropArgs::step)");
        const EdgePick p = pick_backward(a, ext, a.dbg, with_pe);
        if (p.fn == nullptr)
            return fail(GAT_E_UNSUPPORTED, "edge_backward: attention dropout / DropEdge / edge features need the store path (not with GAT_BWD_ATOMICS=1 or without the message scratch)");
        EdgeBwdDropArgs ad;
        if (ext) { static_cast<EdgeBwdArgs&>(ad) = a; ad.drop = dr; ad.pe = pe; ad.gpe = gpe; }
        void* args[] = {ext ? (void*)&ad : (void*)const_cast<EdgeBwdArgs*>(&a)};
        GAT_HIP(hipLaunchKernel(p.fn, dim3((unsigned)a.ga_blocks), dim3(p.block), args, 0, s));
        return launch_bwd_fix(a, s);
    }
    if (a.pos != nullptr) return fail(GAT_E_INVALID, "edge_backward: the generic path has no store mode");
    const int HD = a.H * a.D;
    const size_t lds = (size_t)(3 * a.H + 2 * HD) * sizeof(float);
    if (lds > 64 * 1024) return fail(GAT_E_UNSUPPORTED, "edge_backward: H*D too large for the generic path");
    if (with_pe) hipLaunchKernelGGL(edge_bwd_generic_pe, dim3((unsigned)a.ga_blocks), dim3(64), lds, s, a, dr, pe, gpe);
    else hipLaunchKernelGGL(edge_bwd_generic, dim3((unsigned)a.ga_blocks), dim3(64), lds, s, a, dr);
    GAT_HIP(hipGetLastError());
    return 0;
}

bool edge_last_fused_supported(int32_t H, int32_t D, int32_t C) { return H * D == 64 && D == 8 && C >= 1 && C <= 64; }
int edge_last_fused_blocks(int64_t n_items) {
    const int64_t want = std::max<int64_t>(1, ((n_items + 3) / 4 + 3) / 4);
    const int cap = std::min(resident_blocks((const void*)edge_last_fused_kernel<64, 8, 4>, 256u), kGaPartialRows);
    return (int)std::min<int64_t>(want, cap);
}
int launch_edge_last_fused(const EdgeLastArgs& a, hipStream_t s) {
    if (!edge_last_fused_supported(a.f.H, a.f.D, a.C)) return fail(GAT_E_UNSUPPORTED, "edge_last_fused: shape outside the kernel");
    if (a.f.n_items <= 0) return 0;
    if (a.f.items == nullptr || a.b.pos == nullptr || a.b.stash == nullptr || a.gh_out == nullptr || a.b.ga_blocks < 1 ||
        (a.b.hbits == nullptr && a.b.gfull == nullptr))
        return fail(GAT_E_INVALID, "edge_last_fused: missing buffers");
    hipLaunchKernelGGL((edge_last_fused_kernel<64, 8, 4>), dim3((unsigned)a.b.ga_blocks), dim3(256), 0, s, a);
    GAT_HIP(hipGetLastError());
    return 0;
}
int launch_head_rows(const int4* slot_info, int32_t n_slots, int32_t n_split, const float* Wo, const float* HL, const int32_t* labels,
                     float* gh_out, int32_t gh_stride, int32_t C, int32_t DLAST, hipStream_t s) {
    if (n_split <= 0) return 0;
    if (DLAST > 16) return fail(GAT_E_UNSUPPORTED, "head_rows: D_last > 16");
    hipLaunchKernelGGL(head_rows_kernel, dim3((unsigned)((n_split + 255) / 256)), dim3(256), 0, s, slot_info, n_slots, n_split, Wo, HL,
                       labels, gh_out, gh_stride, C, DLAST);
    GAT_HIP(hipGetLastError());
    return 0;
}

int launch_csr_to_coo(const int32_t* row_ptr, const int32_t* col_idx, int32_t* src, int32_t* dst,
                      int64_t n_rows, int64_t n_edges, int64_t dst_offset, hipStream_t s) {
    if (n_edges <= 0) return 0;
    int64_t blocks = (n_edges + 255) / 256;
    if (blocks > 65536) blocks = 65536;
    hipLaunchKernelGGL(csr_to_coo_kernel, dim3((unsigned)blocks), dim3(256), 0, s, row_ptr, col_idx, src,
                       dst, n_rows, n_edges, (int32_t)dst_offset);
    GAT_HIP(hipGetLastError());
    return 0;
}

static int launch_transpose(const float* src, float* dst, int64_t A_, int64_t B_, hipStream_t s) {
    const int64_t total = A_ * B_;
    if (total <= 0) return 0;
    int64_t blocks = (total + 255) / 256;
    if (blocks > 65536) blocks = 65536;
    hipLaunchKernelGGL(transpose_kernel, dim3((unsigned)blocks), dim3(256), 0, s, src, dst, A_, B_);
    GAT_HIP(hipGetLastError());
    return 0;
}
int launch_transpose_eh_to_he(const float* src_eh, float* dst_he, int64_t E, int32_t H, hipStream_t s) {
    return launch_transpose(src_eh, dst_he, E, H, s);
}
int launch_transpose_he_to_eh(const float* src_he, float* dst_eh, int64_t E, int32_t H, hipStream_t s) {
    return launch_transpose(src_he, dst_eh, H, E, s);
}
int launch_transpose_nh_to_hn(const float* src_nh, float* dst_hn, int64_t N, int32_t H, hipStream_t s) {
    return launch_transpose(src_nh, dst_hn, N, H, s);
}

}
```

graph-attention-network-gatv2-_amd/csrc/gat_internal.h:

```cpp
#pragma once
#include <hip/hip_runtime.h>
#include <cstdint>
#include <cstdio>
#include <string>
#include <vector>

#include "gatv2_abi.h"

namespace gat {

constexpr int kWave = 64;

void set_error(const std::string& msg);
int fail(int code, const std::string& msg);
const char* choice_env(const char* name);

#define GAT_HIP(expr)                                                                     \
    do {                                                                                  \
        hipError_t e__ = (expr);                                                          \
        if (e__ != hipSuccess)                                                            \
            return ::gat::fail((int)e__, std::string(#expr) + ": " + hipGetErrorString(e__)); \
    } while (0)

#define GAT_TRY(expr)                 \
// ... 63 lines not shown
    float* score;
    float* hpre;
    float* hout;
    float* mstat;
    float* zstat;
    int64_t n_rows;
    int64_t n_table;
    int32_t bf16;
    int32_t H, D;
    int32_t is_last;
    float slope;
    const int4* items;
    int64_t n_items;
    const int4* slot_info;
    int32_t n_slots;
    int32_t n_split;
    float* part_acc;
    float* part_mz;
};

constexpr int kSegEdges = 256;
struct WorkList {
    std::vector<int32_t> items;
    std::vector<int32_t> slot_info;
    int64_t n_items = 0;
    int32_t n_slots = 0;
    int32_t n_split = 0;
};
void build_worklist(const int32_t* row_ptr, int64_t n_rows, WorkList& w);
struct LnArgs {
    const float* gamma = nullptr;
    const float* beta = nullptr;
    float eps = 0.f;
};
struct EdgeFwdExtras {
    DropArgs drop;
    const float* res = nullptr;
    const float* bias = nullptr;
    LnArgs ln;
    const float* pe = nullptr;
};
int launch_edge_forward(const EdgeFwdArgs& a, hipStream_t s, const EdgeFwdExtras* extras = nullptr);
struct EdgeFwdExtArgs : EdgeFwdArgs { EdgeFwdExtras x; };

struct EdgeBwdArgs {
    const int32_t* row_ptr;
    const int32_t* col_idx;
    const float* PL;
    const float* PR;
    const float* a;
    const float* alpha;
    const float* mstat;
    const float* zstat;
    const float* hpre;
    const float* g;
    int32_t g_raw;
    const float* gh;
    float* gPL;
    const int32_t* pos;
    float* msg;
    uint32_t* stash;
    uint32_t stash_spare;
    float* gfull;
    int32_t gh_stride;
    int32_t hb_stride;
    uint8_t* hbits;
    float* gPR;
    float* ge;
    float* galpha;
    float* ga_partial;
    int32_t ga_blocks;
    int64_t n_rows;
    int64_t n_table;
    int32_t bf16;
    int32_t H, D;
    float slope;
    const int4* items;
    int64_t n_items;
    const int4* slot_info;
    int32_t n_slots;
    int32_t n_split;
    float* part_acc;
    int32_t dbg;
};
int launch_edge_backward(const EdgeBwdArgs& a, hipStream_t s, const DropArgs* drop = nullptr, const float* pe = nullptr, float* gpe = nullptr);
struct EdgeBwdDropArgs : EdgeBwdArgs { DropArgs drop; const float* pe = nullptr; float* gpe = nullptr; };
struct EdgeLastArgs {
    EdgeFwdArgs f;
    EdgeBwdArgs b;
    const float* Wo;
    const int32_t* labels;
    float* gh_out;
    int32_t C;
};
bool edge_last_fused_supported(int32_t H, int32_t D, int32_t C);
int edge_last_fused_blocks(int64_t n_items);
int launch_edge_last_fused(const EdgeLastArgs& a, hipStream_t s);
int launch_head_rows(const int4* slot_info, int32_t n_slots, int32_t n_split, const float* Wo, const float* HL, const int32_t* labels,
                     float* gh_out, int32_t gh_stride, int32_t C, int32_t DLAST, hipStream_t s);
int edge_stash_words(int32_t H, int32_t D);
constexpr int kGaPartialRows = 2048;
int edge_backward_blocks(const EdgeBwdArgs& a, const DropArgs* drop = nullptr, bool pe = false);
bool edge_fast_path(int32_t H, int32_t D, int64_t n_table);

int build_csc(const int32_t* col_idx, int64_t n_edges, int64_t n_table, int32_t* pos, int32_t* src_ptr,
              int32_t* csrc, hipStream_t s);
struct HeavyList {
    std::vector<int32_t> chunks;
    std::vector<int32_t> heavy;
    int32_t threshold = 0;
    std::vector<int32_t> items;
    int32_t run = 0; int64_t n_runs = 0;
    std::vector<int32_t> open;
    std::vector<int32_t> empty;
};
int build_heavy_list(const int32_t* d_src_ptr, int64_t n_table, int64_t n_edges, HeavyList* out, hipStream_t s, int32_t run = 0);
constexpr int64_t kPullPad = 32;
struct SourceIndex {
    const int32_t* src_ptr = nullptr;
    const int32_t* cdst = nullptr;
    const int32_t* csrc = nullptr;
    int32_t run = 0;
    int64_t n_runs = 0;
    const int4* open = nullptr; int32_t n_open = 0;
    const int32_t* empty = nullptr; int64_t n_empty = 0;
    float* run_part = nullptr;
    const int4* chunks = nullptr; int32_t n_chunks = 0;
    const int4* heavy = nullptr; int32_t n_heavy = 0;
    float* part = nullptr;
    const int4* items = nullptr; int64_t n_items = 0;
    int64_t n_table = 0, n_slots = 0;
    int64_t slot_capacity = 0;
};
constexpr int64_t kRunsMinSlots = 512 << 10;
inline bool short_lists_take_runs(int64_t n_slots, int64_t n_table) { return n_slots < 8 * n_table && n_slots >= kRunsMinSlots; }
int launch_gpl_sum(const SourceIndex& ix, const float* msg, bool msg_bf16, float* gPL, int32_t HD, hipStream_t s);
int build_csc_dst(const int32_t* row_ptr, const int32_t* pos, int32_t* cdst, int64_t n_rows, int64_t n_edges, hipStream_t s);
struct PullArgs {
    const uint32_t* stash; const float* gfull; bool g_bf16; const float* gh; const uint8_t* hbits;
    int32_t gh_stride, hb_stride; const float* a; float slope; float* gPL; int32_t H, D;
};
int launch_gpl_pull(const SourceIndex& ix, const PullArgs& p, hipStream_t s);

int launch_csr_to_coo(const int32_t* row_ptr, const int32_t* col_idx, int32_t* src, int32_t* dst,
                      int64_t n_rows, int64_t n_edges, int64_t table_row0, hipStream_t s);

struct Comm {
    int world = 1, rank = 0;
    virtual ~Comm();
    virtual int all_gather(float* table, int64_t slice, hipStream_t s) = 0;
    virtual int all_gather_part(float* table, int64_t slice, int64_t off, int64_t cnt, hipStream_t s) = 0;
    virtual int reduce_scatter(float* table, int64_t slice, hipStream_t s) = 0;
    virtual int reduce_scatter_bf16(float* table, int64_t slice, hipStream_t s) = 0;
    virtual int all_reduce(float* buf, int64_t n, hipStream_t s) = 0;
    virtual int exchange_rows(const float* sendbuf, const int64_t* cnt_send, float* recvbuf, const int64_t* cnt_recv, int64_t rf, hipStream_t s) = 0;
};
struct HaloPlan {
    int world = 0, rank = 0;
    int64_t max_rows = 0;
    std::vector<int64_t> need_cnt, send_cnt;
    int64_t n_need = 0, n_send = 0, buf_rows = 0;
    int32_t* need_rows = nullptr;
    int32_t* send_rows = nullptr;
    int32_t *arr_ptr = nullptr, *arr_split = nullptr, *arr_pos = nullptr;
    float *sendbuf = nullptr, *recvbuf = nullptr;
    double referenced_fraction = 1.0;
};
int halo_build(Comm* comm, const int32_t* d_col_idx, int64_t n_edges, int64_t n_table, int32_t hd_max, HaloPlan* out, hipStream_t s);
int halo_forward(Comm* comm, const HaloPlan& h, float* table, int64_t rf, hipStream_t s);
int halo_backward(Comm* comm, const HaloPlan& h, float* gPL, int64_t rf, hipStream_t s);
void halo_free(HaloPlan* h);
int comm_unique_id(void* id_out);
int comm_create_rccl(int world, int rank, const void* id_bytes, Comm** out);
int comm_create_host(int world, int rank, const char* shm_name, int64_t bytes_per_rank, Comm** out);

int launch_pack_result(const float* loss, const int32_t* correct, float* dst3, hipStream_t s);
struct ReduceJob { const float* slabs; float* out; int64_t width; int32_t nslabs, HD, F, c_base, block0; };
struct ReduceBatch {
    ReduceJob jobs[8]; int32_t n, blocks;
    const float* loss; const int32_t* correct; float* dst3; float* dst3_host;
    const double* fin_loss; const int32_t* fin_corr; int32_t fin_n; float* fin_loss_out; int32_t* fin_corr_out;
};
void reduce_batch_begin();
void reduce_batch_abort();
void reduce_batch_pack(const float* loss, const int32_t* correct, float* dst3, float* dst3_host);
bool reduce_batch_finalize(const double* loss_partial, const int32_t* correct_partial, int32_t nblocks, float* loss_out, int32_t* correct_out);
int reduce_batch_flush(hipStream_t s);
int launch_reduce_partials_add(const float* partial, int32_t nblocks, int64_t width, float* out,
                               hipStream_t s);

int launch_reduce_gradw(const float* slabs, int32_t ksplit, int32_t HD, int32_t F, int32_t c_base, int32_t M,
                        float* gradW, hipStream_t s);

int64_t resident_blocks(const void* fn, size_t dyn_lds, int threads = 256);

int launch_transpose_eh_to_he(const float* src_eh, float* dst_he, int64_t E, int32_t H, hipStream_t s);
int launch_transpose_he_to_eh(const float* src_he, float* dst_eh, int64_t E, int32_t H, hipStream_t s);
int launch_transpose_nh_to_hn(const float* src_nh, float* dst_hn, int64_t N, int32_t H, hipStream_t s);

enum : int32_t { kPartBoth = 0, kPartLeft = 1, kPartRight = 2 };
int64_t project_scratch_floats(int64_t n_rows, int32_t F, int32_t HD, int32_t part);
int launch_project(const float* X, const float* W, float* PL_rows, float* PR, int64_t n_rows,
                   int32_t F, int32_t HD, int32_t part, bool pl_bf16, float* scratch, int64_t scratch_floats, hipStream_t s, int32_t ldx = 0);
int64_t grad_w_scratch_floats(int64_t n_rows, int32_t F, int32_t HD);
int launch_grad_w(const float* gPL_rows, const float* gPR, const float* X, float* gradW,
                  float* scratch, int64_t n_rows, int32_t F, int32_t HD, int32_t part, hipStream_t s, int32_t ldx = 0);
int launch_grad_x(const float* gPL_rows, const float* gPR, const float* W, const float* hpre_prev,
                  float* gprev, int64_t n_rows, int32_t F, int32_t HD, float slope, hipStream_t s);

int launch_project_res(const float* X, const float* Wres, float* R, int64_t n_rows, int32_t F, int32_t HD, hipStream_t s, int32_t ldx = 0);
int launch_grad_wres(const float* G, const float* X, float* gradWres, float* scratch, int64_t n_rows, int32_t F, int32_t HD,
                     hipStream_t s, int32_t ldx = 0);
int launch_grad_x_res(const float* G, const float* Wres, float* gx, int64_t n_rows, int32_t F, int32_t HD, hipStream_t s);
struct ResBwdArgs {
    const float* hpre; const float* g; const float* gh; const float* res; const float* bias;
    float* G; float* agg; float* partial;
    int64_t n_rows;
    int32_t H, D, gh_stride, g_raw, blocks;
    float slope;
};
constexpr int kResPartialRows = 1024;
int res_backward_blocks(int64_t n_rows, int32_t HD);
int launch_res_backward(const ResBwdArgs& a, hipStream_t s);
// ... 125 lines not shown
```

Before: 2.938 billion edges/s.

## Store backward edge records in edge order and gather them via CSC edge index

Adds a cedge array, built alongside the CSC destination index, that maps each CSC slot back to its CSR edge id. The edge backward kernel can now write stash records in CSR edge order, using contiguous whole-line stores after a quad transpose, instead of scattering them to CSC positions. The gPL pull kernels then gather records through cedge. This trades scattered writes in the edge kernel for indirect reads in the pull. It adds an int per edge of memory and one more index load per pull chunk.

```diff
diff --git a/graph-attention-network-gatv2-_amd/csrc/gat_abi.hip b/graph-attention-network-gatv2-_amd/csrc/gat_abi.hip
--- a/graph-attention-network-gatv2-_amd/csrc/gat_abi.hip
+++ b/graph-attention-network-gatv2-_amd/csrc/gat_abi.hip
@@ -424,7 +424,7 @@
     const char* force = choice_env("GAT_BWD_ATOMICS");
     if ((msg_hd > 0 || stash_words > 0) && E > 0 && !(force && force[0] == '1')) {
         float* m = nullptr;
-        int32_t *src_ptr = nullptr, *cdst = nullptr, *csrc = nullptr;
+        int32_t *src_ptr = nullptr, *cdst = nullptr, *cedge = nullptr, *csrc = nullptr;
         if (hipMalloc((void**)&m, std::max<size_t>((size_t)(E + kPullPad) * msg_hd * (size_t)st_bytes(c), (size_t)(E + kPullPad) * stash_words * sizeof(uint32_t))) == hipSuccess) {
             c->owned.push_back(m);
             if (msg_hd > 0) { c->msg = m; c->msg_hd = msg_hd; }
@@ -435,6 +435,7 @@
                 if (c->layers[L - 1].stash && c->gH != nullptr && c->gh_stride == 16) c->hbits = reinterpret_cast<uint8_t*>(c->gH) + 32;
                 GAT_TRY(dalloc(c, &cdst, E + kPullPad));
                 GAT_HIP(hipMemsetAsync(cdst + E, 0, (size_t)kPullPad * sizeof(int32_t), c->stream));
+                if (!bf16(c)) GAT_TRY(dalloc(c, &cedge, E + kPullPad));
                 GAT_HIP(hipMemsetAsync(reinterpret_cast<uint32_t*>(m) + (size_t)E * stash_words, 0, (size_t)kPullPad * stash_words * sizeof(uint32_t), c->stream));
             }
             GAT_TRY(dalloc(c, &c->csc_pos, E));
@@ -443,9 +444,9 @@
             const int32_t run = run_env >= 0 ? (run_env / 32) * 32 : 64;
             if (run > 0) GAT_TRY(dalloc(c, &csrc, E + kPullPad));
             GAT_TRY(build_csc(c->col_idx, E, T, c->csc_pos, src_ptr, csrc, c->stream));
-            if (cdst) GAT_TRY(build_csc_dst(c->row_ptr, c->csc_pos, cdst, N, E, c->stream));
+            if (cdst) GAT_TRY(build_csc_dst(c->row_ptr, c->csc_pos, cdst, N, E, c->stream, cedge));
             SourceIndex& ix = c->src_index;
-            ix.src_ptr = src_ptr; ix.cdst = cdst; ix.n_table = T; ix.n_slots = E; ix.slot_capacity = E + kPullPad;
+            ix.src_ptr = src_ptr; ix.cdst = cdst; ix.cedge = cedge; ix.n_table = T; ix.n_slots = E; ix.slot_capacity = E + kPullPad;
             HeavyList hl;
             GAT_TRY(build_heavy_list(src_ptr, T, E, &hl, c->stream, run));
             auto upload = [&](auto** d, const std::vector<int32_t>& h, int per) -> int {
@@ -1186,7 +1187,8 @@
     return readout_unpool(c);
 }
 
-struct BwdPlan { EdgeBwdArgs a; bool store, stash, last_g; DropArgs drop; };
+struct BwdPlan { EdgeBwdArgs a; bool store, stash, last_g, edge_order; DropArgs drop; };
+static bool fused_last(gat_ctx* c);
 static int plan_backward_edges(gat_ctx* c, int32_t l, BwdPlan* P) {
     Layer& y = c->layers[l];
     const bool store = c->msg != nullptr && edge_fast_path(y.H, y.D, c->n_table);
@@ -1208,6 +1210,10 @@
     const bool last_g = stash && a.gh != nullptr && c->hbits != nullptr && !bf16(c) && !edge_feat_on(c) && (pull_last >= 0 ? pull_last == 1 : big_rows) &&
                         c->n_rows < ((int64_t)1 << 26);
     a.hbits = last_g ? c->hbits : nullptr;
+    const bool fused = l == c->cfg.num_layers - 1 && fused_last(c);
+    const bool edge_order = stash && !y.ge && c->dbg == 0 && !fused &&
+                            records_take_edge_order(c->src_index, y.H, y.D, !bf16(c), last_g, !last_g || c->gh_stride == 16);
+    a.edge_order = edge_order ? 1 : 0;
     a.items = c->items; a.n_items = c->work.n_items; a.slot_info = c->slot_info; a.n_slots = c->work.n_slots; a.n_split = c->work.n_split;
     a.part_acc = c->part_acc;
     a.dbg = c->dbg;
@@ -1215,7 +1221,7 @@
     a.slope = c->cfg.negative_slope;
     P->drop = drop_args(c, l);
     a.ga_blocks = edge_backward_blocks(a, &P->drop, y.PE != nullptr);
-    P->a = a; P->store = store; P->stash = stash; P->last_g = last_g;
+    P->a = a; P->store = store; P->stash = stash; P->last_g = last_g; P->edge_order = edge_order;
     return 0;
 }
 static int sum_backward_edges(gat_ctx* c, int32_t l, const BwdPlan& P) {
@@ -1224,7 +1230,7 @@
     Scope t(c, GAT_K_GPL_SUM);
     if (P.stash) {
         const PullArgs p{c->stash, c->gfull, bf16(c), P.last_g ? c->gH : nullptr, P.last_g ? c->hbits : nullptr, c->gh_stride, 64,
-                         a_of(c, l), c->cfg.negative_slope, gPL_of(c, l), y.H, y.D};
+                         a_of(c, l), c->cfg.negative_slope, gPL_of(c, l), y.H, y.D, P.edge_order};
         return launch_gpl_pull(c->src_index, p, c->stream);
     }
     return launch_gpl_sum(c->src_index, c->msg, bf16(c), gPL_of(c, l), y.HD, c->stream);
diff --git a/graph-attention-network-gatv2-_amd/csrc/gat_csc.hip b/graph-attention-network-gatv2-_amd/csrc/gat_csc.hip
--- a/graph-attention-network-gatv2-_amd/csrc/gat_csc.hip
+++ b/graph-attention-network-gatv2-_amd/csrc/gat_csc.hip
@@ -332,9 +332,9 @@
     *p = v;
 #endif
 }
-template <int HD, int N, bool BF, int LASTD>
+template <int HD, int N, bool BF, int LASTD, bool EO = false>
 __device__ __forceinline__ typename PullVec<N>::T pull_range(const uint32_t* __restrict__ stash,
-                                                             const int32_t* __restrict__ cdst,
+                                                             const int32_t* __restrict__ cdst, const int32_t* __restrict__ cedge,
                                                              const float* __restrict__ gfull, const uint8_t* __restrict__ hbits, int gh_stride, int hb_stride,
                                                              float slope, int b, int e, int lane,
                                                              typename PullVec<N>::T ac, typename PullVec<N>::T acs) {
@@ -350,16 +350,25 @@
         const int j = i0 + (lane & (CH - 1));
         return cdst[j < e ? j : e - 1];
     };
+    [[maybe_unused]] auto load_edge = [&](int i0) {
+        const int j = i0 + (lane & (CH - 1));
+        return cedge[j < e ? j : e - 1];
+    };
     int dv = load_dst(b);
+    [[maybe_unused]] int ev = 0;
+    if constexpr (EO) ev = load_edge(b);
     for (int i0 = b; i0 < e; i0 += CH) {
         const int dn = (i0 + CH < e) ? load_dst(i0 + CH) : 0;
+        [[maybe_unused]] int en = 0;
+        if constexpr (EO) en = (i0 + CH < e) ? load_edge(i0 + CH) : 0;
         uint32_t w[U];
         V g[U];
 #pragma unroll
         for (int u = 0; u < U; ++u) {
             const int i = i0 + u * G + gidx;
             const int ic = i < e ? i : e - 1;
-            w[u] = stash[(uint64_t)(uint32_t)ic * LPE + cp];
+            if constexpr (EO) w[u] = stash[(uint64_t)(uint32_t)__shfl(ev, u * G + gidx) * LPE + cp];
+            else w[u] = stash[(uint64_t)(uint32_t)ic * LPE + cp];
             const uint32_t drow = (uint32_t)__shfl(dv, u * G + gidx);
             if constexpr (LASTD > 0) {
                 constexpr float inv_heads = 1.0f / (float)(HD / LASTD);
@@ -399,6 +408,7 @@
             acc += (g[u] * al + asel * ge) * keep;
         }
         dv = dn;
+        if constexpr (EO) ev = en;
     }
 #pragma unroll
     for (int off = LPE; off < 64; off <<= 1)
@@ -432,9 +442,9 @@
     if constexpr (N > 2) { r[2] = select_bit<2>(bits, a[2], b[2]); r[3] = select_bit<3>(bits, a[3], b[3]); }
     return r;
 }
-template <int HD, int N, int LASTD, bool TAB>
+template <int HD, int N, int LASTD, bool TAB, bool EO = false>
 __device__ __forceinline__ typename PullVec<N>::T pull_range2(const PullTabs<N>& T, const uint32_t* __restrict__ stash,
-                                                              const int32_t* __restrict__ cdst, const float* __restrict__ gfull,
+                                                              const int32_t* __restrict__ cdst, const int32_t* __restrict__ cedge, const float* __restrict__ gfull,
                                                               const uint8_t* __restrict__ hbits, int b, int e, int lane,
                                                               typename PullVec<N>::T ac, float slope) {
     using V = typename PullVec<N>::T;
@@ -456,15 +466,24 @@
     const char* dp = reinterpret_cast<const char*>(cdst + b);
     const uint32_t doff = (uint32_t)(lane & (CH - 1)) * 4u;
     int dv = *reinterpret_cast<const int32_t*>(dp + doff);
+    [[maybe_unused]] const char* ep = reinterpret_cast<const char*>(cedge + (EO ? b : 0));
+    [[maybe_unused]] int ev = 0;
+    if constexpr (EO) ev = *reinterpret_cast<const int32_t*>(ep + doff);
     for (int rem = e - b; rem > 0; rem -= CH, sp += CH * LPE * 4, dp += CH * 4) {
         const int dn = *reinterpret_cast<const int32_t*>(dp + CH * 4 + doff);
+        [[maybe_unused]] int en = 0;
+        if constexpr (EO) { ep += CH * 4; en = *reinterpret_cast<const int32_t*>(ep + doff); }
         const int d0 = __builtin_amdgcn_readfirstlane(dv);
         uint32_t w[U];
         V g[U];
 #pragma unroll
         for (int u = 0; u < U; ++u) {
             const bool valid = u * G + gidx < rem;
-            const uint32_t ww = *reinterpret_cast<const uint32_t*>(sp + (uint32_t)((u * G + gidx) * LPE + cp) * 4u);
+            uint32_t ww;
+            if constexpr (EO) {
+                const int er = __shfl(ev, u * G + gidx);
+                ww = stash[(uint64_t)(uint32_t)(valid ? er : __builtin_amdgcn_readfirstlane(ev)) * LPE + cp];
+            } else ww = *reinterpret_cast<const uint32_t*>(sp + (uint32_t)((u * G + gidx) * LPE + cp) * 4u);
             int drow = __shfl(dv, u * G + gidx);
             drow = valid ? drow : d0;
             w[u] = valid ? ww : 0u;
@@ -488,6 +507,7 @@
             else acc += select_bits<N>(w[u], ac, acs) * ge;
         }
         dv = dn;
+        if constexpr (EO) ev = en;
     }
 #pragma unroll
     for (int off = LPE; off < 64; off <<= 1)
@@ -495,6 +515,45 @@
         for (int k = 0; k < N; ++k) acc[k] += __shfl_xor(acc[k], off);
     return acc;
 }
+
+#define GAT_PULL_LIST_BODY(BF_, EO_, CEDGE_) \
+    using V = typename PullVec<N>::T; \
+    constexpr int LPE = HD / N; \
+    __shared__ PullTabs<N> tabs; \
+    if constexpr (V2 == 1) pull_tabs_init<N>(tabs, slope, LASTD > 0 ? 1.0f / (float)(HD / (LASTD > 0 ? LASTD : 1)) : 1.0f); \
+    const int lane = threadIdx.x & 63; \
+    const int wave = __builtin_amdgcn_readfirstlane(threadIdx.x >> 6); \
+    const int64_t s = (int64_t)blockIdx.x * (blockDim.x >> 6) + wave; \
+    if (s >= n_table) return; \
+    const int b = __builtin_amdgcn_readfirstlane(src_ptr[s]), e = __builtin_amdgcn_readfirstlane(src_ptr[s + 1]); \
+    if (e - b > kHeavySlots) return;    \
+    const int cp = lane % LPE; \
+    V acc; \
+    if (b < e) { \
+        const V ac = *reinterpret_cast<const V*>(a + cp * N); \
+        if constexpr (V2 != 0) acc = pull_range2<HD, N, LASTD, V2 == 1, EO_>(tabs, stash, cdst, CEDGE_, gfull, hbits, b, e, lane, ac, slope); \
+        else acc = pull_range<HD, N, BF_, LASTD, EO_>(stash, cdst, CEDGE_, gfull, hbits, gh_stride, hb_stride, slope, b, e, lane, ac, ac * slope); \
+    } else { \
+        _Pragma("unroll") \
+        for (int i = 0; i < N; ++i) acc[i] = 0.f; \
+    } \
+    if (lane < LPE) stream_store(reinterpret_cast<V*>(gPL + s * HD + cp * N), acc);
+#define GAT_PULL_CHUNK_BODY(BF_, EO_, CEDGE_) \
+    using V = typename PullVec<N>::T; \
+    constexpr int LPE = HD / N; \
+    __shared__ PullTabs<N> tabs; \
+    if constexpr (V2 == 1) pull_tabs_init<N>(tabs, slope, LASTD > 0 ? 1.0f / (float)(HD / (LASTD > 0 ? LASTD : 1)) : 1.0f); \
+    const int lane = threadIdx.x & 63; \
+    const int wave = __builtin_amdgcn_readfirstlane(threadIdx.x >> 6); \
+    const int k = blockIdx.x * 4 + wave; \
+    if (k >= n_chunks) return; \
+    const int4 ch = chunks[k];    \
+    const int cp = lane % LPE; \
+    const V ac = *reinterpret_cast<const V*>(a + cp * N); \
+    V acc; \
+    if constexpr (V2 != 0) acc = pull_range2<HD, N, LASTD, V2 == 1, EO_>(tabs, stash, cdst, CEDGE_, gfull, hbits, __builtin_amdgcn_readfirstlane(ch.x), __builtin_amdgcn_readfirstlane(ch.y), lane, ac, slope); \
+    else acc = pull_range<HD, N, BF_, LASTD, EO_>(stash, cdst, CEDGE_, gfull, hbits, gh_stride, hb_stride, slope, ch.x, ch.y, lane, ac, ac * slope); \
+    if (lane < LPE) *reinterpret_cast<V*>(part + (int64_t)ch.z * HD + cp * N) = acc;
 
 template <int HD, int N, bool BF, int LASTD, int V2 = 0>
 __global__ __launch_bounds__(256) void gpl_pull_kernel(const int32_t* __restrict__ src_ptr, const uint32_t* __restrict__ stash,
@@ -502,27 +561,15 @@
                                                        const uint8_t* __restrict__ hbits, int gh_stride, int hb_stride,
                                                        const float* __restrict__ a, float slope, float* __restrict__ gPL,
                                                        int64_t n_table, int32_t kHeavySlots) {
-    using V = typename PullVec<N>::T;
-    constexpr int LPE = HD / N;
-    __shared__ PullTabs<N> tabs;
-    if constexpr (V2 == 1) pull_tabs_init<N>(tabs, slope, LASTD > 0 ? 1.0f / (float)(HD / (LASTD > 0 ? LASTD : 1)) : 1.0f);
-    const int lane = threadIdx.x & 63;
-    const int wave = __builtin_amdgcn_readfirstlane(threadIdx.x >> 6);
-    const int64_t s = (int64_t)blockIdx.x * (blockDim.x >> 6) + wave;
-    if (s >= n_table) return;
-    const int b = __builtin_amdgcn_readfirstlane(src_ptr[s]), e = __builtin_amdgcn_readfirstlane(src_ptr[s + 1]);
-    if (e - b > kHeavySlots) return;
-    const int cp = lane % LPE;
-    V acc;
-    if (b < e) {
-        const V ac = *reinterpret_cast<const V*>(a + cp * N);
-        if constexpr (V2 != 0) acc = pull_range2<HD, N, LASTD, V2 == 1>(tabs, stash, cdst, gfull, hbits, b, e, lane, ac, slope);
-        else acc = pull_range<HD, N, BF, LASTD>(stash, cdst, gfull, hbits, gh_stride, hb_stride, slope, b, e, lane, ac, ac * slope);
-    } else {
-#pragma unroll
-        for (int i = 0; i < N; ++i) acc[i] = 0.f;
-    }
-    if (lane < LPE) stream_store(reinterpret_cast<V*>(gPL + s * HD + cp * N), acc);
+    GAT_PULL_LIST_BODY(BF, false, nullptr)
+}
+template <int HD, int N, int LASTD, int V2>
+__global__ __launch_bounds__(256) void gpl_pull_eo_kernel(const int32_t* __restrict__ src_ptr, const uint32_t* __restrict__ stash,
+                                                          const int32_t* __restrict__ cdst, const float* __restrict__ gfull,
+                                                          const uint8_t* __restrict__ hbits, int gh_stride, int hb_stride,
+                                                          const float* __restrict__ a, float slope, float* __restrict__ gPL,
+                                                          int64_t n_table, int32_t kHeavySlots, const int32_t* __restrict__ cedge) {
+    GAT_PULL_LIST_BODY(false, true, cedge)
 }
 
 template <int HD, int N, bool BF, int LASTD, int V2 = 0>
@@ -531,22 +578,18 @@
                                                              const float* __restrict__ gfull, const uint8_t* __restrict__ hbits,
                                                              int gh_stride, int hb_stride, const float* __restrict__ a,
                                                              float slope, float* __restrict__ part) {
-    using V = typename PullVec<N>::T;
-    constexpr int LPE = HD / N;
-    __shared__ PullTabs<N> tabs;
-    if constexpr (V2 == 1) pull_tabs_init<N>(tabs, slope, LASTD > 0 ? 1.0f / (float)(HD / (LASTD > 0 ? LASTD : 1)) : 1.0f);
-    const int lane = threadIdx.x & 63;
-    const int wave = __builtin_amdgcn_readfirstlane(threadIdx.x >> 6);
-    const int k = blockIdx.x * 4 + wave;
-    if (k >= n_chunks) return;
-    const int4 ch = chunks[k];
-    const int cp = lane % LPE;
-    const V ac = *reinterpret_cast<const V*>(a + cp * N);
-    V acc;
-    if constexpr (V2 != 0) acc = pull_range2<HD, N, LASTD, V2 == 1>(tabs, stash, cdst, gfull, hbits, __builtin_amdgcn_readfirstlane(ch.x), __builtin_amdgcn_readfirstlane(ch.y), lane, ac, slope);
-    else acc = pull_range<HD, N, BF, LASTD>(stash, cdst, gfull, hbits, gh_stride, hb_stride, slope, ch.x, ch.y, lane, ac, ac * slope);
-    if (lane < LPE) *reinterpret_cast<V*>(part + (int64_t)ch.z * HD + cp * N) = acc;
-}
+    GAT_PULL_CHUNK_BODY(BF, false, nullptr)
+}
+template <int HD, int N, int LASTD, int V2>
+__global__ __launch_bounds__(256) void gpl_pull_chunk_eo_kernel(const int4* __restrict__ chunks, int32_t n_chunks,
+                                                                const uint32_t* __restrict__ stash, const int32_t* __restrict__ cdst,
+                                                                const float* __restrict__ gfull, const uint8_t* __restrict__ hbits,
+                                                                int gh_stride, int hb_stride, const float* __restrict__ a,
+                                                                float slope, float* __restrict__ part, const int32_t* __restrict__ cedge) {
+    GAT_PULL_CHUNK_BODY(false, true, cedge)
+}
+#undef GAT_PULL_LIST_BODY
+#undef GAT_PULL_CHUNK_BODY
 
 template <int HD, int N, bool BF, int LASTD>
 __global__ __launch_bounds__(256) void gpl_pull3_kernel(const int4* __restrict__ items, int64_t n_items,
@@ -867,7 +910,7 @@
 }
 
 __global__ __launch_bounds__(256) void csc_dst_kernel(const int32_t* __restrict__ row_ptr, const int32_t* __restrict__ pos,
-                                                     int32_t* __restrict__ cdst, int64_t n_rows, int64_t n_edges) {
+                                                     int32_t* __restrict__ cdst, int64_t n_rows, int64_t n_edges, int32_t* __restrict__ cedge) {
     const int64_t stride = (int64_t)gridDim.x * blockDim.x;
     for (int64_t e = (int64_t)blockIdx.x * blockDim.x + threadIdx.x; e < n_edges; e += stride) {
         int64_t lo = 0, hi = n_rows;
@@ -875,16 +918,24 @@
             const int64_t mid = (lo + hi) >> 1;
             if ((int64_t)row_ptr[mid] <= e) lo = mid; else hi = mid;
         }
-        cdst[pos[e]] = (int32_t)lo;
-    }
-}
-
-}
-
-int build_csc_dst(const int32_t* row_ptr, const int32_t* pos, int32_t* cdst, int64_t n_rows, int64_t n_edges, hipStream_t s) {
+        const int32_t p = pos[e];
+        cdst[p] = (int32_t)lo;
+        if (cedge != nullptr) cedge[p] = (int32_t)e;
+    }
+}
+__global__ __launch_bounds__(64) void fill_kernel(int32_t* v, int32_t n, int32_t value) {
+    if ((int)threadIdx.x < n) v[threadIdx.x] = value;
+}
+
+}
+
+int build_csc_dst(const int32_t* row_ptr, const int32_t* pos, int32_t* cdst, int64_t n_rows, int64_t n_edges, hipStream_t s, int32_t* cedge) {
+    static_assert(kPullPad <= 64, "one block fills the padding");
     if (n_edges <= 0) return 0;
+    if (cedge != nullptr)
+        hipLaunchKernelGGL(fill_kernel, dim3(1), dim3(64), 0, s, cedge + n_edges, (int32_t)kPullPad, (int32_t)n_edges);
     const int64_t blocks = std::min<int64_t>((n_edges + 255) / 256, 65536);
-    hipLaunchKernelGGL(csc_dst_kernel, dim3((unsigned)blocks), dim3(256), 0, s, row_ptr, pos, cdst, n_rows, n_edges);
+    hipLaunchKernelGGL(csc_dst_kernel, dim3((unsigned)blocks), dim3(256), 0, s, row_ptr, pos, cdst, n_rows, n_edges, cedge);
     GAT_HIP(hipGetLastError());
     return 0;
 }
@@ -916,6 +967,27 @@
 static int gpl_bf16_group_env() {
     static const int v = [] { const char* e = choice_env("GAT_GPL_BF16_GROUP"); return e ? (e[0] == '0' ? 0 : 1) : -1; }();
     return v;
+}
+static int stash_order_env() {
+    static const int v = [] { const char* e = choice_env("GAT_STASH_ORDER"); return e ? (e[0] == '0' ? 0 : e[0] == 'h' ? 1 : e[0] == 'l' ? 2 : 3) : -1; }();
+    return v;
+}
+
+PullForm pull_form(const SourceIndex& ix, int32_t lpe, bool records64) {
+    const bool padded = ix.slot_capacity >= ix.n_slots + kPullPad;
+    const int runs_env = pull_runs_env(), groups_env = pull_groups_env();
+    const bool runs_ok = padded && ix.csrc != nullptr && ix.run % lpe == 0 && records64;
+    if (runs_ok && (runs_env >= 0 ? runs_env == 1 : (groups_env < 0 && short_lists_take_runs(ix.n_slots, ix.n_table)))) return kPullRuns;
+    const bool groups = groups_env >= 0 ? groups_env == 1 : (ix.n_slots < 8 * ix.n_table && ix.n_items >= 32768);
+    return (ix.items != nullptr && groups) ? kPullItems : kPullLists;
+}
+bool records_take_edge_order(const SourceIndex& ix, int32_t H, int32_t D, bool fp32, bool node_records, bool records64) {
+    const int words = edge_stash_words(H, D);
+    if (!fp32 || words == 0 || ix.cedge == nullptr || !edge_backward_groups(H, D)) return false;
+    if (pull_form(ix, words, records64) != kPullLists) return false;
+    const int env = stash_order_env();
+    if (env >= 0) return (env >> (node_records ? 1 : 0)) & 1;
+    return node_records ? kEdgeOrderLast : kEdgeOrderHidden;
 }
 
 namespace {
@@ -943,10 +1015,10 @@
 GplPick pick_pull(const SourceIndex& ix, const PullArgs& A, bool padded) {
     constexpr int LPE = HD / N, G = 64 / LPE;
     const int wpb = gpl_waves_env() ? gpl_waves_env() : 1;
-    const int runs_env = pull_runs_env(), groups_env = pull_groups_env();
     const bool records64 = LASTD == 0 || (A.gh_stride == 16 && A.hb_stride == 64);
-    const bool runs_ok = padded && ix.csrc != nullptr && ix.run % LPE == 0 && records64;
-    if (runs_ok && (runs_env >= 0 ? runs_env == 1 : (groups_env < 0 && short_lists_take_runs(ix.n_slots, ix.n_table)))) {
+    const PullForm form = pull_form(ix, LPE, records64);
+    if (A.edge_order && !records_take_edge_order(ix, A.H, A.D, !BF, LASTD > 0, records64)) return {};
+    if (form == kPullRuns) {
         constexpr int U = LPE % 8 == 0 ? 8 : 4;
         const int u_env = pull_u_env();
         if constexpr (LPE == 16 && !BF) {
@@ -955,8 +1027,7 @@
         }
         return pick_runs(ix, GAT_K(gpl_pull_runs_kernel<HD, N, BF, LASTD, U>), G);
     }
-    const bool groups = groups_env >= 0 ? groups_env == 1 : (ix.n_slots < 8 * ix.n_table && ix.n_items >= 32768);
-    if (ix.items != nullptr && groups) {
+    if (form == kPullItems) {
         const int64_t quads = (ix.n_items + G - 1) / G;
         return {GAT_K(gpl_pull3_kernel<HD, N, BF, LASTD>), GplPick::kItems, nullptr, (unsigned)((quads + 3) / 4)};
     }
@@ -965,6 +1036,11 @@
     const int v2 = (padded && !BF && records64) ? v2_want : 0;
     const unsigned grid = (unsigned)((ix.n_table + wpb - 1) / wpb), block = 64u * wpb;
     if constexpr (!BF) {
+        if (A.edge_order) {
+            if (v2 == 1) return {GAT_K(gpl_pull_eo_kernel<HD, N, LASTD, 1>), GplPick::kLists, GAT_K(gpl_pull_chunk_eo_kernel<HD, N, LASTD, 1>), grid, block};
+            if (v2 == 2) return {GAT_K(gpl_pull_eo_kernel<HD, N, LASTD, 2>), GplPick::kLists, GAT_K(gpl_pull_chunk_eo_kernel<HD, N, LASTD, 2>), grid, block};
+            return {GAT_K(gpl_pull_eo_kernel<HD, N, LASTD, 0>), GplPick::kLists, GAT_K(gpl_pull_chunk_eo_kernel<HD, N, LASTD, 0>), grid, block};
+        }
         if (v2 == 1) return {GAT_K(gpl_pull_kernel<HD, N, BF, LASTD, 1>), GplPick::kLists, GAT_K(gpl_pull_chunk_kernel<HD, N, BF, LASTD, 1>), grid, block};
         if (v2 == 2) return {GAT_K(gpl_pull_kernel<HD, N, BF, LASTD, 2>), GplPick::kLists, GAT_K(gpl_pull_chunk_kernel<HD, N, BF, LASTD, 2>), grid, block};
     }
@@ -1042,13 +1118,13 @@
     const bool padded = ix.slot_capacity >= ix.n_slots + kPullPad;
     const bool last = A.gh != nullptr && A.hbits != nullptr;
     GplPick p = pick_pull_pass(ix, A, last, padded);
-    if (p.fn == nullptr) return fail(GAT_E_UNSUPPORTED, "gpl_pull: no stash path for this (H, D)");
+    if (p.fn == nullptr) return fail(GAT_E_UNSUPPORTED, A.edge_order ? "gpl_pull: records in edge order where the record-order rule gives the scattered layout" : "gpl_pull: no stash path for this (H, D)");
     SourceIndex x = ix;
     PullArgs q = A;
     const float* g = last ? A.gh : A.gfull;
     int32_t hs = heavy_slots(ix.n_slots);
-    void* lists[] = {&x.src_ptr, &q.stash, &x.cdst, &g, &q.hbits, &q.gh_stride, &q.hb_stride, &q.a, &q.slope, &q.gPL, &x.n_table, &hs};
-    void* chunk[] = {&x.chunks, &x.n_chunks, &q.stash, &x.cdst, &g, &q.hbits, &q.gh_stride, &q.hb_stride, &q.a, &q.slope, &x.part};
+    void* lists[] = {&x.src_ptr, &q.stash, &x.cdst, &g, &q.hbits, &q.gh_stride, &q.hb_stride, &q.a, &q.slope, &q.gPL, &x.n_table, &hs, &x.cedge};
+    void* chunk[] = {&x.chunks, &x.n_chunks, &q.stash, &x.cdst, &g, &q.hbits, &q.gh_stride, &q.hb_stride, &q.a, &q.slope, &x.part, &x.cedge};
     void* items[] = {&x.items, &x.n_items, &q.stash, &x.cdst, &g, &q.hbits, &q.gh_stride, &q.hb_stride, &q.a, &q.slope, &q.gPL, &x.part};
     void* runs[] = {&q.stash, &x.cdst, &g, &q.hbits, &q.a, &q.slope, &q.gPL, &p.rd};
     return run_pick(ix, p, p.form == GplPick::kRuns ? runs : p.form == GplPick::kItems ? items : lists, chunk, A.gPL, A.H * A.D, s);
diff --git a/graph-attention-network-gatv2-_amd/csrc/gat_edge_kernels.hip b/graph-attention-network-gatv2-_amd/csrc/gat_edge_kernels.hip
--- a/graph-attention-network-gatv2-_amd/csrc/gat_edge_kernels.hip
+++ b/graph-attention-network-gatv2-_amd/csrc/gat_edge_kernels.hip
@@ -564,6 +564,18 @@
 #else
     *p = v;
 #endif
+}
+__device__ __forceinline__ void quad_transpose4(uint32_t (&a)[4], int t) {
+    const bool o1 = (t & 1) != 0, o2 = (t & 2) != 0;
+    auto swap = [](uint32_t& lo, uint32_t& hi, bool odd, auto ctrl) {
+        const uint32_t x = odd ? lo : hi;
+        const uint32_t y = (uint32_t)__builtin_amdgcn_update_dpp(0, (int)x, decltype(ctrl)::value, 0xF, 0xF, true);
+        if (odd) lo = y; else hi = y;
+    };
+    swap(a[0], a[1], o1, std::integral_constant<int, 0xB1>{});
+    swap(a[2], a[3], o1, std::integral_constant<int, 0xB1>{});
+    swap(a[0], a[2], o2, std::integral_constant<int, 0x4E>{});
+    swap(a[1], a[3], o2, std::integral_constant<int, 0x4E>{});
 }
 template <int HD, int N, bool BF>
 __device__ __forceinline__ void store_row_n(float* __restrict__ msg, int slot, int cp, vnf<N> v) {
@@ -1015,9 +1027,10 @@
     edge_bwd2_body<HD, D, N, DBG, false, true>(A);
 }
 
-template <int HD, int D, int N, int DBG = 0, bool BF = false, bool MSG = false, bool DROP = false, bool PE = false>
+template <int HD, int D, int N, int DBG = 0, bool BF = false, bool MSG = false, bool DROP = false, bool PE = false, bool EO = false, bool LINES = false>
 __global__ __launch_bounds__(256) __attribute__((amdgpu_waves_per_eu(DROP ? 3 : 4, 8))) void edge_bwd3_kernel(BwdArgsT<DROP> A) {
     static_assert(DROP || !PE, "the edge term travels in the extended argument struct");
+    static_assert(!EO || (!MSG && !BF && DBG == 0), "edge order: fp32 records");
     constexpr int LPE = HD / N, G = 64 / LPE, DL = D / N, H = HD / D;
     constexpr int U = 4;
     static_assert((MSG || DL == 2) && LPE >= U, "records: two lanes per head (one carries alpha, the other ge)");
@@ -1026,6 +1039,14 @@
     const int wave = __builtin_amdgcn_readfirstlane(threadIdx.x >> 6);
     const int cp = lane % LPE, gidx = lane / LPE;
     const int c = N * cp;
+    static_assert(!LINES || (EO && LPE % 4 == 0 && U == 4), "whole-line stores: edge order, quads of lanes inside a group");
+    [[maybe_unused]] auto store_lines = [&](int b, int e, int stp, uint32_t (&pw)[U]) {
+        uint32_t o[4] = {pw[0], pw[1], pw[2], pw[3]};
+        quad_transpose4(o, cp & 3);
+        const int j = b + stp * U + (cp & 3);
+        const uint32_t rec = (j >= b && j < e) ? (uint32_t)j : A.stash_spare;
+        stream_store(reinterpret_cast<uint4*>(A.stash + ((uint64_t)rec * LPE + (cp & ~3))), make_uint4(o[0], o[1], o[2], o[3]));
+    };
     const vnf<N> ac = *reinterpret_cast<const vnf<N>*>(A.a + c);
     const vnf<N> acs = ac * A.slope;
     const vnf<N> ac2 = ac * kLog2e;
@@ -1046,7 +1067,7 @@
             j = j < e ? j : e - 1;
             j = j > 0 ? j : 0;
             srcv = A.col_idx[j];
-            posv = (DBG == 2) ? j : A.pos[j];
+            posv = (DBG == 2 || EO) ? j : A.pos[j];
             if constexpr (DBG >= 15 && DBG <= 18) {
                 constexpr uint32_t K = DBG == 15 ? 64u : DBG == 16 ? 512u : DBG == 17 ? 4096u : 32768u;
                 const uint32_t per = A.stash_spare / K;
@@ -1151,6 +1172,8 @@
                 const int j0 = b + (st > 0 ? st - 1 : 0) * U;
                 uint4 w4 = make_uint4(pend_w[0], pend_w[1], pend_w[2], pend_w[3]);
                 *reinterpret_cast<uint4*>(A.stash + (uint64_t)(uint32_t)(j0 < e ? j0 : 0) * LPE + cp * 4) = w4;
+            } else if constexpr (LINES) {
+                store_lines(b, e, st - 1, pend_w);
             } else if constexpr (DBG != 1) {
 #pragma unroll
                 for (int u = 0; u < U; ++u) stream_store(&A.stash[(uint64_t)pend_s[u] * LPE + cp], pend_w[u]);
@@ -1209,6 +1232,8 @@
 #pragma unroll
                 for (int u = 0; u < U; ++u) store_row_n<HD, N, BF>(A.msg, (int)pend_s[u], cp, pend_m[u]);
             }
+        } else if constexpr (LINES) {
+            store_lines(b, e, nst - 1, pend_w);
         } else if constexpr (DBG != 1 && DBG != 3) {
 #pragma unroll
             for (int u = 0; u < U; ++u) stream_store(&A.stash[(uint64_t)pend_s[u] * LPE + cp], pend_w[u]);
@@ -1877,11 +1902,16 @@
     for (const auto& sh : kEdgeShapes) if (sh.HD == HD && sh.D == D) return true;
     return false;
 }
+constexpr bool kStashLines = true;
 constexpr int stash_n(int HD, int D) { return (D == 8 && HD >= 32) ? 4 : (D == 4 ? 2 : 0); }
 template <int HD, int D> constexpr int stash_n() { return stash_n(HD, D); }
 
 static bool row_groups() {
     static const bool v = [] { const char* e = choice_env("GAT_ROWGROUP"); return !(e && e[0] == '0'); }();
+    return v;
+}
+static bool stash_lines() {
+    static const bool v = [] { const char* e = choice_env("GAT_STASH_LINES"); return e ? e[0] != '0' : kStashLines; }();
     return v;
 }
 static bool packed_layout() {
@@ -1953,14 +1983,24 @@
 EdgePick pick_bwd(const EdgeBwdArgs& a, bool drop, int dbg, bool pe) {
     constexpr int N3 = stash_n<HD, D>(), N2 = (HD >= 32 && D % 4 == 0) ? 4 : 2;
     const bool store = a.pos != nullptr && a.msg != nullptr, taps = a.ge != nullptr, stash = a.stash != nullptr && !taps;
+    [[maybe_unused]] const bool eo = a.edge_order != 0 && stash && store && !BF && N3 != 0 && row_groups() && dbg == 0;
+    [[maybe_unused]] const bool lines = eo && stash_lines();
     if (drop) {
         if (!store) return {};
         if (pe) {
             if (taps) return {GAT_K(edge_bwd_kernel<HD, D, true, true, 0, BF, true, true>)};
+            if constexpr (N3 != 0 && !BF) {
+                if (lines) return {GAT_K(edge_bwd3_kernel<HD, D, N3, 0, false, false, true, true, true, true>)};
+                if (eo) return {GAT_K(edge_bwd3_kernel<HD, D, N3, 0, false, false, true, true, true>)};
+            }
             if constexpr (N3 != 0) return {stash ? GAT_K(edge_bwd3_kernel<HD, D, N3, 0, BF, false, true, true>) : GAT_K(edge_bwd3_kernel<HD, D, N3, 0, BF, true, true, true>)};
             else return {GAT_K(edge_bwd2_kernel<HD, D, N2, 0, BF, false, true, true>)};
         }
         if (taps) return {GAT_K(edge_bwd_kernel<HD, D, true, true, 0, BF, true>)};
+        if constexpr (N3 != 0 && !BF) {
+            if (lines) return {GAT_K(edge_bwd3_kernel<HD, D, N3, 0, false, false, true, false, true, true>)};
+            if (eo) return {GAT_K(edge_bwd3_kernel<HD, D, N3, 0, false, false, true, false, true>)};
+        }
         if constexpr (N3 != 0) return {stash ? GAT_K(edge_bwd3_kernel<HD, D, N3, 0, BF, false, true>) : GAT_K(edge_bwd3_kernel<HD, D, N3, 0, BF, true, true>)};
         else return {GAT_K(edge_bwd2_kernel<HD, D, N2, 0, BF, false, true>)};
     }
@@ -1985,6 +2025,10 @@
     }
 #endif
     if constexpr (N3 != 0) {
+        if constexpr (!BF) {
+            if (lines) return {GAT_K(edge_bwd3_kernel<HD, D, N3, 0, false, false, false, false, true, true>)};
+            if (eo) return {GAT_K(edge_bwd3_kernel<HD, D, N3, 0, false, false, false, false, true>)};
+        }
         if (stash) return {(BF || row_groups()) ? GAT_K(edge_bwd3_kernel<HD, D, N3, 0, BF>) : GAT_K(edge_bwd2s_kernel<HD, D, N3>)};
         if (msg_rows && row_groups() && group_msg()) {
 #ifdef GAT_EXPERIMENTS
@@ -2061,6 +2105,7 @@
     const int n = edge_shape_listed(H * D, D) ? stash_n(H * D, D) : 0;
     return n ? H * D / n : 0;
 }
+bool edge_backward_groups(int32_t H, int32_t D) { return edge_shape_listed(H * D, D) && stash_n(H * D, D) != 0 && row_groups(); }
 
 int launch_edge_forward(const EdgeFwdArgs& a, hipStream_t s, const EdgeFwdExtras* extras) {
     if (a.n_rows <= 0) return 0;
@@ -2115,6 +2160,8 @@
         if (a.stash != nullptr && a.ge == nullptr && (a.gfull == nullptr || a.pos == nullptr))
             return fail(GAT_E_INVALID, "edge_backward: stash path needs gfull and pos");
         if (ext && dr.step == nullptr) return fail(GAT_E_INVALID, "edge_backward: the extended kernels read the device counter (DropArgs::step)");
+        if (a.edge_order && !(a.stash != nullptr && a.ge == nullptr && !a.bf16 && a.dbg == 0 && edge_backward_groups(a.H, a.D)))
+            return fail(GAT_E_INVALID, "edge_backward: records in edge order need the fp32 group-per-row record kernel");
         const EdgePick p = pick_backward(a, ext, a.dbg, with_pe);
         if (p.fn == nullptr)
             return fail(GAT_E_UNSUPPORTED, "edge_backward: attention dropout / DropEdge / edge features need the store path (not with GAT_BWD_ATOMICS=1 or without the message scratch)");
diff --git a/graph-attention-network-gatv2-_amd/csrc/gat_internal.h b/graph-attention-network-gatv2-_amd/csrc/gat_internal.h
--- a/graph-attention-network-gatv2-_amd/csrc/gat_internal.h
+++ b/graph-attention-network-gatv2-_amd/csrc/gat_internal.h
@@ -169,6 +169,7 @@
     int32_t n_split;
     float* part_acc;
     int32_t dbg;
+    int32_t edge_order;
 };
 int launch_edge_backward(const EdgeBwdArgs& a, hipStream_t s, const DropArgs* drop = nullptr, const float* pe = nullptr, float* gpe = nullptr);
 struct EdgeBwdDropArgs : EdgeBwdArgs { DropArgs drop; const float* pe = nullptr; float* gpe = nullptr; };
@@ -206,6 +207,7 @@
 struct SourceIndex {
     const int32_t* src_ptr = nullptr;
     const int32_t* cdst = nullptr;
+    const int32_t* cedge = nullptr;
     const int32_t* csrc = nullptr;
     int32_t run = 0;
     int64_t n_runs = 0;
@@ -221,11 +223,17 @@
 };
 constexpr int64_t kRunsMinSlots = 512 << 10;
 inline bool short_lists_take_runs(int64_t n_slots, int64_t n_table) { return n_slots < 8 * n_table && n_slots >= kRunsMinSlots; }
+enum PullForm : int32_t { kPullLists, kPullItems, kPullRuns };
+PullForm pull_form(const SourceIndex& ix, int32_t lpe, bool records64);
+bool edge_backward_groups(int32_t H, int32_t D);
+constexpr bool kEdgeOrderHidden = true, kEdgeOrderLast = false;
+bool records_take_edge_order(const SourceIndex& ix, int32_t H, int32_t D, bool fp32, bool node_records, bool records64);
 int launch_gpl_sum(const SourceIndex& ix, const float* msg, bool msg_bf16, float* gPL, int32_t HD, hipStream_t s);
-int build_csc_dst(const int32_t* row_ptr, const int32_t* pos, int32_t* cdst, int64_t n_rows, int64_t n_edges, hipStream_t s);
+int build_csc_dst(const int32_t* row_ptr, const int32_t* pos, int32_t* cdst, int64_t n_rows, int64_t n_edges, hipStream_t s, int32_t* cedge = nullptr);
 struct PullArgs {
     const uint32_t* stash; const float* gfull; bool g_bf16; const float* gh; const uint8_t* hbits;
     int32_t gh_stride, hb_stride; const float* a; float slope; float* gPL; int32_t H, D;
+    bool edge_order = false;
 };
 int launch_gpl_pull(const SourceIndex& ix, const PullArgs& p, hipStream_t s);
 
```

New measurement: 2.995 billion edges/s (median of 6 runs). 1.02x the previous value.
